# edwinb-ai/MolecularDynamics.jl

Hardware: AMD Instinct MI355X
Metric: particle-steps/sec + achieved HBM GB/s, 1M LJ particles rho=0.897, 1/2/4/8 GPUs (higher is better)
Workload: dtype f64; 1 GPU; BASELINE configs[2]: N=1048576 monodisperse LJ 3D rho=0.897 r_cut=2.5 dt=0.001 NVT Bussi tau=0.1 kT=1.4737, per GPU; particles_per_gpu=1048576, parallelism=1 GPU, step_loop=fused (k_step_tile: one launch per step + k_finalize), global_particles=1048576, tiled_force_kernel=True, max_tile_halo=2081, energies_every_step=False, thermo_frequency=2589

## Files before the change

### include/mdhip.h

```cpp
#ifndef MDHIP_H
#define MDHIP_H

#include <stdint.h>

#ifdef __cplusplus
extern "C" {
#endif

typedef struct md_ctx md_ctx;

enum { MD_POT_LJ = 0, MD_POT_PSEUDOHS = 1, MD_POT_POLYDISPERSE = 2, MD_POT_LJ_MODIFIED = 3, MD_POT_CUSTOM = 100 };

enum { MD_NVE = 0, MD_NVT = 1 };

int md_create(int dim, int64_t n_particles, const double *box, double list_cutoff, int device_id, md_ctx **out);
int md_destroy(md_ctx *ctx);

const char *md_last_error(md_ctx *ctx);

int md_set_potential(md_ctx *ctx, int kind, const double *params, int nparams);

int md_set_potential_source(md_ctx *ctx, const char *hip_src, const char *entry_name, const double *params,
                            int nparams);

int md_set_skin(md_ctx *ctx, double skin);

int md_set_inner_skin(md_ctx *ctx, double inner_skin);

int md_upload(md_ctx *ctx, const double *x, const double *v, const double *f, const int32_t *images,
              const double *diameters);
int md_download(md_ctx *ctx, double *x, double *v, double *f, int32_t *images);

int md_compute_forces(md_ctx *ctx, double *energy, double *virial);

int md_neighbor_pairs(md_ctx *ctx, int32_t *pairs, int64_t cap, int64_t *count);

int md_run(md_ctx *ctx, int64_t nsteps, double dt, int ensemble, double tau, double nf, const double *ktemp,
           const double *r1, const double *r2, double *uwk);

int md_fire_minimize(md_ctx *ctx, int64_t max_steps, double tol, double dt_initial, double dt_max, double alpha0,
                     double f_inc, double f_dec, int nmin, int64_t *steps, int *converged, double *energy,
                     double *f_rms);

int md_run_brownian(md_ctx *ctx, int64_t nsteps, double dt, double ktemp, uint64_t seed, int64_t first_step,
                    int64_t virial_every, double *out );

int md_snapshot_begin(md_ctx *ctx);
int md_snapshot_end(md_ctx *ctx, double *x, int32_t *images);

int md_rdf_setup(md_ctx *ctx, double r_max, int nbins);
int md_rdf_sample(md_ctx *ctx);
int md_rdf_read(md_ctx *ctx, int64_t *counts, int64_t *nsamples);
int md_rdf_reset(md_ctx *ctx);

int md_dyn_setup(md_ctx *ctx, int nslots, int nrows, const double *q, int nq, double r_max, int nbins);
int md_dyn_origin(md_ctx *ctx, int slot);
int md_dyn_sample(md_ctx *ctx, const int32_t *slots, const int32_t *rows, int count);
int md_dyn_read(md_ctx *ctx, int64_t *nsamples, double *sums, int64_t *hist);
int md_dyn_reset(md_ctx *ctx);

int md_sq_setup(md_ctx *ctx, const int32_t *n, int nvec, int nslots, int nrows);
int md_sq_sample(md_ctx *ctx, int add_static, const int32_t *slots, const int32_t *rows, int count, int origin_slot);
int md_sq_rho(md_ctx *ctx, double *rho);
int md_sq_read(md_ctx *ctx, int64_t *nstatic, double *s2, int64_t *nsamples, double *corr);
int md_sq_reset(md_ctx *ctx);

int md_kinetic(md_ctx *ctx, double *kinetic);

int md_scale_velocities(md_ctx *ctx, double s);

typedef struct {
    int64_t steps;
    int64_t rebuilds;
    int64_t violations;
    int64_t n_ghost;
    int64_t max_neighbors;
    double avg_neighbors;
    int64_t force_launches;
    double force_ms;
    int64_t max_halo;
    int64_t tiled;
    int64_t prunes;
    int64_t kickdrift_launches;
    double kickdrift_ms;
    int64_t fused;
    int64_t walked_outer;
    int64_t walked_inner;
    int64_t prune_launches_timed;
    double prune_ms;
    int64_t rebuilds_timed;
    double rebuild_ms;
    int64_t fused_build;
} md_stats;
int md_profile(md_ctx *ctx, int enable);
int md_get_stats(md_ctx *ctx, md_stats *out);

int md_create_domain(int dim, int64_t n_global, int64_t n_cap, const double *box, double list_cutoff,
                     int device_id, int rank, int nranks, md_ctx **out);
int md_dom_set_uniform(md_ctx *ctx, int uniform, double sigma);
int md_dom_upload(md_ctx *ctx, int64_t n_own, const int32_t *ids, const double *x, const double *v, const double *f,
                  const int32_t *images, const double *diameters);
int md_dom_download(md_ctx *ctx, int64_t cap, int64_t *n_own, int32_t *ids, double *x, double *v, double *f,
                    int32_t *images);
int md_dom_migrate_pack(md_ctx *ctx, int64_t *nsend );
int md_dom_migrate_unpack(md_ctx *ctx, const int64_t *nrecv );
int md_dom_halo_pack(md_ctx *ctx, int64_t *nsend );
int md_dom_halo_unpack(md_ctx *ctx, const int64_t *nrecv );
int md_dom_build(md_ctx *ctx);
int md_dom_set_step_buffers(md_ctx *ctx, void *send_left, void *send_right, void *recv_left, void *recv_right,
                            int64_t capacity_doubles);
int md_dom_get_sendbuf(md_ctx *ctx, int side, int64_t ndoubles, void *dst, int dst_is_device);
int md_dom_put_recvbuf(md_ctx *ctx, int side, int64_t ndoubles, const void *src, int src_is_device);
int md_dom_step_begin(md_ctx *ctx, double dt, int *violated);
int md_dom_step_end(md_ctx *ctx, double dt, int want_uw, double *uwk);
int md_dom_forces(md_ctx *ctx, double dt, int kick, int want_uw, double *uwk);
int md_dom_set_scale(md_ctx *ctx, double scale);
int md_dom_counts(md_ctx *ctx, int64_t *out );

int md_set_stream(md_ctx *ctx, void *hip_stream);
int md_dom_async_begin(md_ctx *ctx, int64_t nsteps, double dt, int ensemble, double tau, double nf, const double *ktemp,
                       const double *r1, const double *r2, int64_t prune_interval, void *flag_dev ,
                       void *kuw_dev );
int md_dom_step_a(md_ctx *ctx, double dt, int step);
int md_dom_step_b(md_ctx *ctx, double dt, int step, int want_uw);
int md_dom_step_c(md_ctx *ctx, int step, int want_uw);
int md_dom_async_end(md_ctx *ctx, int apply_pending_scale, int32_t *first_viol, double *uwk, double *info );

int md_dom_comm_unique_id(const char *rccl_path, void *id128);
int md_dom_comm_init(md_ctx *ctx, const char *rccl_path, const void *id128);
int md_dom_rebuild(md_ctx *ctx);
int md_dom_run_window(md_ctx *ctx, int64_t nsteps, double dt, int ensemble, double tau, double nf, const double *ktemp,
                      const double *r1, const double *r2, int report_last, int apply_pending_scale,
                      int64_t prune_interval, int32_t *first_viol, double *uwk, double *info );
int md_dom_enable_pruning(md_ctx *ctx, int on);
int md_dom_max_disp0(md_ctx *ctx, double *d0);
int md_dom_invalidate_inner(md_ctx *ctx);

const char *md_version(void);

#ifdef __cplusplus
}
#endif
#endif
```

### moleculardynamics/jl_amd/_lib.py

```python
import ctypes as C
import os

_HERE = os.path.dirname(os.path.abspath(__file__))
SO_PATH = os.path.join(_HERE, "csrc", "libmdhip.so")

MD_POT_LJ, MD_POT_PSEUDOHS, MD_POT_POLYDISPERSE, MD_POT_LJ_MODIFIED, MD_POT_CUSTOM = 0, 1, 2, 3, 100
MD_NVE, MD_NVT = 0, 1

EXPORTS = [
    "md_create", "md_destroy", "md_last_error", "md_set_potential", "md_set_potential_source", "md_set_skin",
    "md_set_inner_skin",
    "md_upload", "md_download", "md_snapshot_begin", "md_snapshot_end", "md_compute_forces", "md_neighbor_pairs", "md_run", "md_kinetic",
    "md_scale_velocities", "md_profile", "md_get_stats", "md_version", "md_fire_minimize", "md_run_brownian",
    "md_create_domain", "md_dom_set_uniform", "md_dom_upload", "md_dom_download", "md_dom_migrate_pack",
    "md_dom_migrate_unpack", "md_dom_halo_pack", "md_dom_halo_unpack", "md_dom_build", "md_dom_get_sendbuf",
    "md_dom_put_recvbuf", "md_dom_set_step_buffers", "md_dom_step_begin", "md_dom_step_end", "md_dom_forces", "md_dom_set_scale",
    "md_dom_counts", "md_set_stream", "md_dom_async_begin", "md_dom_step_a", "md_dom_step_b", "md_dom_step_c",
    "md_dom_async_end", "md_dom_comm_unique_id", "md_dom_comm_init", "md_dom_run_window", "md_dom_rebuild",
    "md_dom_enable_pruning", "md_dom_max_disp0", "md_dom_invalidate_inner",
    "md_rdf_setup", "md_rdf_sample", "md_rdf_read", "md_rdf_reset",
    "md_dyn_setup", "md_dyn_origin", "md_dyn_sample", "md_dyn_read", "md_dyn_reset",
    "md_sq_setup", "md_sq_sample", "md_sq_rho", "md_sq_read", "md_sq_reset",
]


class MdStats(C.Structure):
    _fields_ = [("steps", C.c_int64), ("rebuilds", C.c_int64), ("violations", C.c_int64), ("n_ghost", C.c_int64),
                ("max_neighbors", C.c_int64), ("avg_neighbors", C.c_double), ("force_launches", C.c_int64),
                ("force_ms", C.c_double), ("max_halo", C.c_int64), ("tiled", C.c_int64), ("prunes", C.c_int64),
                ("kickdrift_launches", C.c_int64), ("kickdrift_ms", C.c_double), ("fused", C.c_int64),
                ("walked_outer", C.c_int64), ("walked_inner", C.c_int64), ("prune_launches_timed", C.c_int64),
                ("prune_ms", C.c_double), ("rebuilds_timed", C.c_int64), ("rebuild_ms", C.c_double),
                ("fused_build", C.c_int64)]


class MdhipError(RuntimeError):
    pass


_lib = None


def load():
    global _lib
    if _lib is not None:
        return _lib
    if not os.path.exists(SO_PATH):
        raise MdhipError(
            f"{SO_PATH} not found: build it with `python -c 'import __graft_entry__ as g; g.build()'` or "
            "`make -C moleculardynamics/jl_amd/csrc`. There is no CPU fallback.")
    L = C.CDLL(SO_PATH)
    vp, dp, ip = C.c_void_p, C.POINTER(C.c_double), C.POINTER(C.c_int32)
    L.md_create.argtypes = [C.c_int, C.c_int64, dp, C.c_double, C.c_int, C.POINTER(vp)]
    L.md_create.restype = C.c_int
    L.md_destroy.argtypes = [vp]
    L.md_destroy.restype = C.c_int
    L.md_last_error.argtypes = [vp]
    L.md_last_error.restype = C.c_char_p
    L.md_set_potential.argtypes = [vp, C.c_int, dp, C.c_int]
    L.md_set_potential.restype = C.c_int
    L.md_set_potential_source.argtypes = [vp, C.c_char_p, C.c_char_p, dp, C.c_int]
    L.md_set_potential_source.restype = C.c_int
    L.md_set_skin.argtypes = [vp, C.c_double]
    L.md_set_skin.restype = C.c_int
    L.md_set_inner_skin.argtypes = [vp, C.c_double]
    L.md_set_inner_skin.restype = C.c_int
    L.md_upload.argtypes = [vp, dp, dp, dp, ip, dp]
    L.md_upload.restype = C.c_int
    L.md_download.argtypes = [vp, dp, dp, dp, ip]
    L.md_download.restype = C.c_int
    L.md_snapshot_begin.argtypes = [vp]
    L.md_snapshot_begin.restype = C.c_int
    L.md_snapshot_end.argtypes = [vp, dp, ip]
    L.md_snapshot_end.restype = C.c_int
    L.md_compute_forces.argtypes = [vp, dp, dp]
    L.md_compute_forces.restype = C.c_int
    L.md_neighbor_pairs.argtypes = [vp, ip, C.c_int64, C.POINTER(C.c_int64)]
    L.md_neighbor_pairs.restype = C.c_int
    L.md_run.argtypes = [vp, C.c_int64, C.c_double, C.c_int, C.c_double, C.c_double, dp, dp, dp, dp]
    L.md_run.restype = C.c_int
    L.md_kinetic.argtypes = [vp, dp]
    L.md_kinetic.restype = C.c_int
    L.md_scale_velocities.argtypes = [vp, C.c_double]
    L.md_scale_velocities.restype = C.c_int
    L.md_profile.argtypes = [vp, C.c_int]
    L.md_profile.restype = C.c_int
    L.md_get_stats.argtypes = [vp, C.POINTER(MdStats)]
    L.md_get_stats.restype = C.c_int
    L.md_version.argtypes = []
    L.md_version.restype = C.c_char_p
    i64p = C.POINTER(C.c_int64)
    L.md_create_domain.argtypes = [C.c_int, C.c_int64, C.c_int64, dp, C.c_double, C.c_int, C.c_int, C.c_int,
                                   C.POINTER(vp)]
    L.md_run_brownian.restype = C.c_int
    L.md_run_brownian.argtypes = [vp, C.c_int64, C.c_double, C.c_double, C.c_uint64, C.c_int64, C.c_int64, dp]
    L.md_fire_minimize.restype = C.c_int
    L.md_fire_minimize.argtypes = [vp, C.c_int64, C.c_double, C.c_double, C.c_double, C.c_double, C.c_double, C.c_double,
                                   C.c_int, i64p, C.POINTER(C.c_int), dp, dp]
    L.md_dom_set_uniform.argtypes = [vp, C.c_int, C.c_double]
    L.md_dom_upload.argtypes = [vp, C.c_int64, ip, dp, dp, dp, ip, dp]
    L.md_dom_download.argtypes = [vp, C.c_int64, i64p, ip, dp, dp, dp, ip]
    L.md_dom_migrate_pack.argtypes = [vp, i64p]
    L.md_dom_migrate_unpack.argtypes = [vp, i64p]
    L.md_dom_halo_pack.argtypes = [vp, i64p]
    L.md_dom_halo_unpack.argtypes = [vp, i64p]
    L.md_dom_build.argtypes = [vp]
    L.md_dom_rebuild.argtypes = [vp]
    L.md_dom_get_sendbuf.argtypes = [vp, C.c_int, C.c_int64, C.c_void_p, C.c_int]
    L.md_dom_put_recvbuf.argtypes = [vp, C.c_int, C.c_int64, C.c_void_p, C.c_int]
    L.md_dom_set_step_buffers.argtypes = [vp, C.c_void_p, C.c_void_p, C.c_void_p, C.c_void_p, C.c_int64]
    L.md_dom_step_begin.argtypes = [vp, C.c_double, C.POINTER(C.c_int)]
    L.md_dom_step_end.argtypes = [vp, C.c_double, C.c_int, dp]
    L.md_dom_forces.argtypes = [vp, C.c_double, C.c_int, C.c_int, dp]
    L.md_dom_set_scale.argtypes = [vp, C.c_double]
    L.md_dom_counts.argtypes = [vp, i64p]
    L.md_set_stream.argtypes = [vp, C.c_void_p]
    L.md_dom_async_begin.argtypes = [vp, C.c_int64, C.c_double, C.c_int, C.c_double, C.c_double, dp, dp, dp, C.c_int64,
                                     C.c_void_p, C.c_void_p]
    L.md_dom_step_a.argtypes = [vp, C.c_double, C.c_int]
    L.md_dom_step_b.argtypes = [vp, C.c_double, C.c_int, C.c_int]
    L.md_dom_step_c.argtypes = [vp, C.c_int, C.c_int]
    L.md_dom_async_end.argtypes = [vp, C.c_int, C.POINTER(C.c_int32), dp, dp]
    L.md_dom_comm_unique_id.argtypes = [C.c_char_p, C.c_void_p]
    L.md_dom_comm_init.argtypes = [vp, C.c_char_p, C.c_void_p]
    L.md_dom_run_window.argtypes = [vp, C.c_int64, C.c_double, C.c_int, C.c_double, C.c_double, dp, dp, dp, C.c_int, C.c_int,
                                    C.c_int64, C.POINTER(C.c_int32), dp, dp]
    L.md_dom_enable_pruning.argtypes = [vp, C.c_int]
    L.md_dom_max_disp0.argtypes = [vp, dp]
    L.md_dom_invalidate_inner.argtypes = [vp]
    L.md_rdf_setup.argtypes = [vp, C.c_double, C.c_int]
    L.md_rdf_setup.restype = C.c_int
    L.md_rdf_sample.argtypes = [vp]
    L.md_rdf_sample.restype = C.c_int
    L.md_rdf_read.argtypes = [vp, i64p, i64p]
    L.md_rdf_read.restype = C.c_int
    L.md_rdf_reset.argtypes = [vp]
    L.md_rdf_reset.restype = C.c_int
    L.md_dyn_setup.argtypes = [vp, C.c_int, C.c_int, dp, C.c_int, C.c_double, C.c_int]
    L.md_dyn_setup.restype = C.c_int
    L.md_dyn_origin.argtypes = [vp, C.c_int]
    L.md_dyn_origin.restype = C.c_int
    L.md_dyn_sample.argtypes = [vp, ip, ip, C.c_int]
    L.md_dyn_sample.restype = C.c_int
    L.md_dyn_read.argtypes = [vp, i64p, dp, i64p]
    L.md_dyn_read.restype = C.c_int
    L.md_dyn_reset.argtypes = [vp]
    L.md_dyn_reset.restype = C.c_int
    L.md_sq_setup.argtypes = [vp, ip, C.c_int, C.c_int, C.c_int]
    L.md_sq_setup.restype = C.c_int
    L.md_sq_sample.argtypes = [vp, C.c_int, ip, ip, C.c_int, C.c_int]
    L.md_sq_sample.restype = C.c_int
    L.md_sq_rho.argtypes = [vp, dp]
    L.md_sq_rho.restype = C.c_int
    L.md_sq_read.argtypes = [vp, i64p, dp, i64p, dp]
    L.md_sq_read.restype = C.c_int
    L.md_sq_reset.argtypes = [vp]
    L.md_sq_reset.restype = C.c_int
    for name in EXPORTS:
        if name.startswith("md_dom_") or name in ("md_create_domain", "md_set_stream"):
            getattr(L, name).restype = C.c_int
    _lib = L
    return L
```

### moleculardynamics/jl_amd/csrc/md_kernels.hpp

```cpp
#ifndef MD_RTC
#pragma once
#include <hip/hip_runtime.h>
#include <stdint.h>
#else
typedef __hip_internal::uint64_t uint64_t;
typedef __hip_internal::uint32_t uint32_t;
typedef __hip_internal::int32_t int32_t;
typedef __hip_internal::uint16_t uint16_t;
#endif

#define MD_BLOCK 256
#define MD_WAVE 64
#define MD_SENTINEL_POS 1.0e100
#define MD_VAL_SRC_BITS 26
#define MD_VAL_SRC_MASK ((1u << MD_VAL_SRC_BITS) - 1u)
#define MD_NO_VIOLATION 0x7fffffff

enum { POT_LJ = 0, POT_PSEUDOHS = 1, POT_POLYDISPERSE = 2, POT_LJ_MOD = 3, POT_CUSTOM = 100 };

struct DevState {
    double4 *pos;
    double *v[3];
    double *f[3];
    int32_t *img[3];
    int32_t *id;
    double *x0[3];
    double *x1[3];
    double boxL[3];
    int tric;
    double cellA[9];
};

struct BoxGrid {
    double L[3], invL[3];
    double lo[3];
    int selfimg[3];
    double inv_cell[3];
    int nc[3];
    int ncx[3];
    int bd[3];
    int nb[3];
    int n_int_cells;
    int id_bits, cell_bits;
    int tric;
    double A[9], Ainv[9];
};

struct PotParams {
    double p[8];
    double c2;
    uint32_t c2_k;
    uint32_t pad_;
    double sig2u;
    double sig_u;
    double c48, c24, c4;
    double ljA, ljB;
};

struct Scalars {
    double U, W, K, scale, T;
    unsigned long long max_disp2_bits;
    int first_viol;
    int overflow;
    unsigned long long pair_count;
    int hmax;
    int halo_overflow;
    int dbg_rmax, dbg_smax;
    unsigned long long d1max2_bits;
    int comm_error;
};

__device__ __forceinline__ double md_rcp(double a)
{
    double r = __builtin_amdgcn_rcp(a);
    double e = __builtin_fma(-a, r, 1.0);
    r = __builtin_fma(r, e, r);
    e = __builtin_fma(-a, r, 1.0);
    r = __builtin_fma(r, e, r);
    return r;
}

__device__ __forceinline__ double md_rcp1(double a)
{
    double r = __builtin_amdgcn_rcp(a);
    double e = __builtin_fma(-a, r, 1.0);
    return __builtin_fma(r, e, r);
}

__device__ __forceinline__ double mask_d2(double d2, bool hit)
{
    int hi = __double2hiint(d2);
    int lo = __double2loint(d2);
    hi = hit ? hi : 0x7fe00000;
    return __hiloint2double(hi, lo);
}

template <int D>
__device__ __forceinline__ double d2_ref(double dx, double dy, double dz)
{
#pragma clang fp contract(off)
    double a = dx * dx;
    double b = dy * dy;
    double r = a + b;
    if constexpr (D == 3) {
        double c = dz * dz;
        r = r + c;
    }
    return r;
}

template <int D>
__device__ __forceinline__ void frac_of(double x, double y, double z, const double *Ainv, double *fr)
{
#pragma clang fp contract(off)
#pragma unroll
    for (int r = 0; r < 3; ++r) {
        if (r < D) {
            double a = Ainv[r * 3 + 0] * x + Ainv[r * 3 + 1] * y;
            if constexpr (D == 3) a = a + Ainv[r * 3 + 2] * z;
            fr[r] = a;
        } else {
            fr[r] = 0.0;
        }
    }
}
template <int D>
__device__ __forceinline__ bool wrap_general(double &x, double &y, double &z, const double *A, const double *Ainv, int32_t *dn)
{
#pragma clang fp contract(off)
    double fr[3];
    frac_of<D>(x, y, z, Ainv, fr);
    bool out = false;
#pragma unroll
    for (int r = 0; r < D; ++r) out = out || fr[r] < 0.0 || fr[r] >= 1.0;
    dn[0] = dn[1] = dn[2] = 0;
    if (!out) return false;
    double fm[3] = {0.0, 0.0, 0.0};
#pragma unroll
    for (int r = 0; r < D; ++r) {
        double nn = floor(fr[r]);
        fm[r] = fr[r] - nn;
        dn[r] = (int32_t)nn;
    }
    double o[3] = {x, y, z};
#pragma unroll
    for (int r = 0; r < D; ++r) {
        double a = A[r * 3 + 0] * fm[0] + A[r * 3 + 1] * fm[1];
        if constexpr (D == 3) a = a + A[r * 3 + 2] * fm[2];
        o[r] = a;
    }
    x = o[0];
    y = o[1];
    if constexpr (D == 3) z = o[2];
    return true;
}
__device__ __forceinline__ void shift_xyz(double &x, double &y, double &z, uint32_t code, const double *L, int tric, const double *A)
{
#pragma clang fp contract(off)
    (void)L;
    (void)tric;
    const uint32_t sx = code & 3u, sy = (code >> 2) & 3u, sz = (code >> 4) & 3u;
    const double s0 = sx == 1u ? 1.0 : (sx == 2u ? -1.0 : 0.0);
    const double s1 = sy == 1u ? 1.0 : (sy == 2u ? -1.0 : 0.0);
    const double s2 = sz == 1u ? 1.0 : (sz == 2u ? -1.0 : 0.0);
    x = x + ((s0 * A[0] + s1 * A[1]) + s2 * A[2]);
    y = y + ((s0 * A[3] + s1 * A[4]) + s2 * A[5]);
    z = z + ((s0 * A[6] + s1 * A[7]) + s2 * A[8]);
}

__device__ __forceinline__ size_t row_off(int r, int lane) { return ((size_t)(r >> 2) * 64 + lane) * 4 + (r & 3); }

__device__ __forceinline__ double md_ipow(double x, int n)
{
    double r = 1.0;
    while (n) {
        if (n & 1) r *= x;
        x *= x;
        n >>= 1;
    }
    return r;
// ... 264 lines not shown
{
#pragma unroll
    for (int c = 0; c < 3; ++c) {
        e[c] = 0;
        b[c] = 0;
    }
    int cc3[3];
    cell_coords<D>(p, g, cc3);
#pragma unroll
    for (int c = 0; c < D; ++c) {
        double xc = pos_get(p, c);
        if (is_xh && !g.selfimg[c]) {
            e[c] = (xc < g.lo[c]) ? 0 : g.nc[c] + 1;
            continue;
        }
        int cc = cc3[c];
        e[c] = cc + 1;
        if (g.selfimg[c]) b[c] = (cc == 0) ? 1 : ((cc == g.nc[c] - 1) ? 2 : 0);
    }
}

template <int D>
__global__ void __launch_bounds__(MD_BLOCK)
    k_wrap_count(int n_src, int n_own_src, DevState s, BoxGrid g, const int32_t *__restrict__ alive,
                 int32_t *__restrict__ nimg)
{
    int i = blockIdx.x * blockDim.x + threadIdx.x;
    if (i >= n_src) return;
    if (i == 0) nimg[n_src] = 0;
    if (alive && !alive[i]) {
        nimg[i] = 0;
        return;
    }
    bool is_xh = i >= n_own_src;
    double4 p = s.pos[i];
    if (!is_xh) {
        bool moved = false;
        if (g.tric) {
            int32_t dn[3];
            moved = wrap_general<D>(p.x, p.y, p.z, g.A, g.Ainv, dn);
            if (moved) {
#pragma unroll
                for (int c = 0; c < D; ++c) s.img[c][i] += dn[c];
            }
        } else {
#pragma unroll
            for (int c = 0; c < D; ++c) {
                double xc = pos_get(p, c);
                if (xc < 0.0 || xc >= g.L[c]) {
                    double frac = g.invL[c] * xc;
                    double nn = floor(frac);
                    double fm = frac - nn;
                    s.img[c][i] += (int32_t)nn;
                    xc = g.L[c] * fm;
                    pos_set(p, c, xc);
                    moved = true;
                }
            }
        }
        if (moved) s.pos[i] = p;
    }
    int e[3], b[3];
    source_cells<D>(p, is_xh, g, e, b);
    int cnt = 1;
#pragma unroll
    for (int c = 0; c < D; ++c)
        if (b[c]) cnt *= 2;
    nimg[i] = cnt;
}

template <int D>
__global__ void __launch_bounds__(MD_BLOCK)
    k_emit(int n_src, int n_own_src, DevState s, BoxGrid g, const int32_t *__restrict__ alive,
           const int32_t *__restrict__ img_off, uint64_t *__restrict__ keys, uint32_t *__restrict__ vals,
           int32_t *__restrict__ cell_start, int32_t *__restrict__ cell_end, int ncell1)
{
    int i = blockIdx.x * blockDim.x + threadIdx.x;
    for (int j = i; j < ncell1; j += gridDim.x * blockDim.x) {
        cell_start[j] = 0;
        cell_end[j] = 0;
    }
    if (i >= n_src) return;
    if (alive && !alive[i]) return;
    bool is_xh = i >= n_own_src;
    double4 p = s.pos[i];
    int eb[3], b[3];
    source_cells<D>(p, is_xh, g, eb, b);
    uint64_t idv = (uint64_t)(uint32_t)s.id[i];
    uint64_t gbit = 1ull << (g.id_bits + g.cell_bits);
    int slot = img_off[i];
    for (int m = 0; m < (1 << D); ++m) {
        bool ok = true;
        uint32_t code = 0;
        int e[3] = {eb[0], eb[1], eb[2]};
#pragma unroll
        for (int c = 0; c < D; ++c) {
            if ((m >> c) & 1) {
                if (b[c] == 0) ok = false;
                e[c] = (b[c] == 1) ? g.nc[c] + 1 : 0;
                code |= (uint32_t)b[c] << (2 * c);
            }
        }
        if (!ok) continue;
        bool ghost = is_xh || m != 0;
        keys[slot] = (ghost ? gbit : 0ull) | ((uint64_t)ext_linear(e, g) << g.id_bits) | idv;
        vals[slot] = (uint32_t)i | (code << MD_VAL_SRC_BITS);
        ++slot;
    }
}

__device__ __forceinline__ double4 shifted(double4 p, uint32_t code, const BoxGrid &g)
{
    if (code) shift_xyz(p.x, p.y, p.z, code, g.L, g.tric, g.A);
    return p;
}

__device__ __forceinline__ void reset_flags(Scalars *sc)
{
    sc->first_viol = MD_NO_VIOLATION;
    sc->max_disp2_bits = 0ull;
    sc->overflow = 0;
    sc->hmax = 0;
    sc->halo_overflow = 0;
    sc->dbg_rmax = 0;
    sc->dbg_smax = 0;
    sc->d1max2_bits = 0ull;
}

template <int D>
__global__ void __launch_bounds__(MD_BLOCK)
    k_gather(int n, int next, DevState so, DevState sn, BoxGrid g, const uint64_t *__restrict__ keys,
             const uint32_t *__restrict__ vals, int32_t *__restrict__ newslot, int32_t *__restrict__ gsrc,
             uint32_t *__restrict__ gcode, int32_t *__restrict__ cell_start, int32_t *__restrict__ cell_end,
             Scalars *sc)
{
    int k = blockIdx.x * blockDim.x + threadIdx.x;
    if (k >= next) return;
    if (k == 0) reset_flags(sc);
    uint64_t key = keys[k];
    uint32_t val = vals[k];
    int src = (int)(val & MD_VAL_SRC_MASK);
    uint32_t code = val >> MD_VAL_SRC_BITS;
    double4 p = shifted(so.pos[src], code, g);
    sn.pos[k] = p;
    sn.id[k] = so.id[src];
    if (k < n) {
#pragma unroll
        for (int c = 0; c < D; ++c) {
            sn.v[c][k] = so.v[c][src];
            sn.f[c][k] = so.f[c][src];
            sn.img[c][k] = so.img[c][src];
            sn.x0[c][k] = pos_get(p, c);
        }
    } else {
        gsrc[k - n] = src;
        gcode[k - n] = code;
    }
    if (code == 0u) newslot[src] = k;
    uint64_t cmask = (1ull << (g.cell_bits + 1)) - 1ull;
    int ce = (int)((key >> g.id_bits) & cmask);
    int cprev = (k > 0) ? (int)((keys[k - 1] >> g.id_bits) & cmask) : -1;
    int cellmask = (1 << g.cell_bits) - 1;
    if (ce != cprev) {
        cell_start[ce & cellmask] = k;
        if (k > 0) cell_end[cprev & cellmask] = k;
    }
    if (k == next - 1) cell_end[ce & cellmask] = next;
}

__global__ void __launch_bounds__(MD_BLOCK)
    k_ghost_owner(int nghost, const int32_t *__restrict__ gsrc, const int32_t *__restrict__ newslot,
                  int32_t *__restrict__ gowner)
{
    int gi = blockIdx.x * blockDim.x + threadIdx.x;
    if (gi >= nghost) return;
    gowner[gi] = newslot[gsrc[gi]];
}

__global__ void __launch_bounds__(MD_BLOCK)
    k_halo_virtualize(int n, uint32_t *__restrict__ halo, int hcap, const int32_t *__restrict__ halo_count,
                      const int32_t *__restrict__ gowner, const uint32_t *__restrict__ gcode)
{
    uint32_t *hl = halo + (size_t)blockIdx.x * hcap;
    int H = halo_count[blockIdx.x];
    for (int h = threadIdx.x; h < H; h += blockDim.x) {
        uint32_t e = hl[h];
        if (e >= (uint32_t)n) hl[h] = (uint32_t)gowner[e - n] | (gcode[e - n] << 26);
    }
}

template <int D>
__global__ void __launch_bounds__(MD_BLOCK)
    k_ghost_update(int n, int nghost, DevState s, BoxGrid g, const int32_t *__restrict__ gowner,
                   const uint32_t *__restrict__ gcode, const Scalars *__restrict__ sc, int step)
{
    int gi = blockIdx.x * blockDim.x + threadIdx.x;
    if (gi >= nghost) return;
    if (sc->first_viol <= step) return;
    s.pos[n + gi] = shifted(s.pos[gowner[gi]], gcode[gi], g);
}

template <int D>
__global__ void __launch_bounds__(MD_BLOCK)
    k_build_list(int n, DevState s, BoxGrid g, double rl2, const int32_t *__restrict__ cell_start,
                 const int32_t *__restrict__ cell_end, uint32_t *__restrict__ nlist, int maxn,
                 int32_t *__restrict__ nneigh, int32_t *__restrict__ nmax_tile, uint32_t sentinel, Scalars *sc)
{
    int k = blockIdx.x * blockDim.x + threadIdx.x;
    bool active = k < n;
    int lane = threadIdx.x & 63;
    int tile = k >> 6;
    uint32_t *row = nlist + ((size_t)tile * maxn) * 64 + lane;
    const double4 *__restrict__ P = s.pos;
    int cnt = 0;
    if (active) {
        double4 pi = P[k];
        int ec[3];
        cell_coords<D>(pi, g, ec);
#pragma unroll
        for (int c = 0; c < D; ++c) ec[c] += 1;
        int z0 = (D == 3) ? -1 : 0, z1 = (D == 3) ? 1 : 0;
        for (int dz = z0; dz <= z1; ++dz)
            for (int dy = -1; dy <= 1; ++dy)
                for (int dx = -1; dx <= 1; ++dx) {
                    int e[3] = {ec[0] + dx, ec[1] + dy, (D == 3) ? ec[2] + dz : 0};
                    int cell = ext_linear(e, g);
                    int js = cell_start[cell], je = cell_end[cell];
                    for (int j = js; j < je; ++j) {
                        double4 pj = P[j];
                        double ddx = pj.x - pi.x;
                        double ddy = pj.y - pi.y;
                        double d2 = ddx * ddx;
                        d2 = __builtin_fma(ddy, ddy, d2);
                        if constexpr (D == 3) {
                            double ddz = pj.z - pi.z;
                            d2 = __builtin_fma(ddz, ddz, d2);
                        }
                        if (d2 <= rl2 && j != k) {
                            if (cnt < maxn) row[(size_t)cnt * 64] = (uint32_t)j;
                            ++cnt;
                        }
                    }
                }
        nneigh[k] = cnt;
        if (cnt > maxn) {
            atomicOr(&sc->overflow, 1);
            cnt = maxn;
        }
    }
    int m = wave_max_i(cnt);
    m = (m + 3) & ~3;
    if (m > maxn) m = maxn;
    for (int t = cnt; t < m; ++t) row[(size_t)t * 64] = sentinel;
    if (lane == 0) nmax_tile[tile] = m;
}

template <int D, int POT, bool UNIFORM, bool WANT_UW, bool KICK>
__global__ void __launch_bounds__(MD_BLOCK)
    k_force(int n, DevState s, PotParams pp, const uint32_t *__restrict__ nlist, int maxn,
            const int32_t *__restrict__ nmax_tile, double dt, double *__restrict__ partials, int nblk_total,
            const Scalars *__restrict__ sc, int step)
{
    __shared__ double red[16];
    if (sc->first_viol <= step) return;
    int bid = xcd_remap(blockIdx.x, gridDim.x);
    int k = bid * MD_BLOCK + threadIdx.x;
    bool active = k < n;
    int kk = active ? k : n - 1;
    int lane = threadIdx.x & 63;
    int tile = kk >> 6;
    const uint32_t *row = nlist + ((size_t)tile * maxn) * 64 + lane;
    int m = nmax_tile[tile];
    const double4 *__restrict__ P = s.pos;
    double4 pi = P[kk];
    double fx = 0.0, fy = 0.0, fz = 0.0, us = 0.0, ws = 0.0;
    for (int r = 0; r < m; r += 4) {
        uint32_t j[4];
#pragma unroll
        for (int q = 0; q < 4; ++q) j[q] = row[(size_t)(r + q) * 64];
        double4 pj[4];
#pragma unroll
        for (int q = 0; q < 4; ++q) pj[q] = P[j[q]];
#pragma unroll
        for (int q = 0; q < 4; ++q) {
            double dx = pj[q].x - pi.x;
            double dy = pj[q].y - pi.y;
            double dz = 0.0;
            if constexpr (D == 3) dz = pj[q].z - pi.z;
            double d2 = d2_ref<D>(dx, dy, dz);
            bool hit = d2 < pp.c2;
            double d2m = mask_d2(d2, hit);
            double u = 0.0, fpr;
            pair_eval<POT, UNIFORM, WANT_UW>(d2m, pi.w, pj[q].w, pp, u, fpr);
            fx = __builtin_fma(-fpr, dx, fx);
            fy = __builtin_fma(-fpr, dy, fy);
            if constexpr (D == 3) fz = __builtin_fma(-fpr, dz, fz);
            if constexpr (WANT_UW) {
                us += u;
                ws = __builtin_fma(fpr, hit ? d2 : 0.0, ws);
            }
        }
    }
    double ke = 0.0;
    if (active) {
        s.f[0][k] = fx;
        s.f[1][k] = fy;
// ... 85 lines not shown
            if (run < hcap) halo[(size_t)tile * hcap + run] = key;
            ++run;
        }
    }
    if (tid == 0) {
        halo_count[tile] = H;
        atomicMax(&sc->hmax, H);
        if (H > hcap || (H + 1) * rs > 65535) atomicOr(&sc->halo_overflow, 1);
    }
    __syncthreads();
    uint16_t *row16 = nlist16 + ((size_t)wt * maxn) * 64;
    for (int r = 0; r < m; ++r) {
        uint32_t j = row[(size_t)r * 64];
        uint32_t loc;
        if (j == sentinel) {
            loc = (uint32_t)H;
        } else {
            uint32_t h = (j * 2654435761u) >> (32 - MD_HT_BITS);
            while (keys[h] != j) h = (h + 1) & (MD_HT - 1);
            loc = vals[h];
        }
        row16[row_off(r, lane)] = (uint16_t)(loc * (uint32_t)rs);
    }
}

#ifndef MD_RTC
#include "md_build_tile.hpp"
#endif

struct PruneRow {
    unsigned char *base;
    unsigned off;
};
__device__ __forceinline__ void prune_append(unsigned entry, PruneRow &pr, unsigned long long &acc, int &cin)
{
    unsigned lo = (unsigned)acc, hi = (unsigned)(acc >> 32);
    lo = __builtin_amdgcn_alignbit(hi, lo, 16);
    hi = __builtin_amdgcn_alignbit(entry, hi, 16);
    acc = ((unsigned long long)hi << 32) | lo;
    ++cin;
    if ((cin & 3) == 0) {
        *(unsigned long long *)(pr.base + pr.off) = acc;
        pr.off += 512u;
    }
}

template <int D, int POT, bool UNIFORM, bool WANT_UW, bool PRUNE, int NQ>
__device__ __forceinline__ void tile_pair_block(const unsigned char *smem, const unsigned (&o)[NQ], const double4 &pi,
                                                const PotParams &pp, PruneRow &rin64, double rin2,
                                                unsigned long long &acc, int &cin, double &fx, double &fy, double &fz,
                                                double &us, double &ws, const uint16_t *remap8)
{
    double xj[NQ], yj[NQ], zj[NQ], wj[NQ];
#pragma unroll
    for (int q = 0; q < NQ; ++q) {
        typedef const volatile __attribute__((address_space(3))) double lds_cvd;
        if constexpr (!UNIFORM && D == 3) {
            typedef double md_d2 __attribute__((ext_vector_type(2)));
            typedef const __attribute__((address_space(3))) md_d2 lds_d2;
            lds_d2 *r2 = (lds_d2 *)(smem + o[q]);
            md_d2 a = r2[0], b = r2[1];
            xj[q] = a.x;
            yj[q] = a.y;
            zj[q] = b.x;
            wj[q] = b.y;
        } else {
            lds_cvd *rec = (lds_cvd *)(smem + o[q]);
            xj[q] = rec[0];
            yj[q] = rec[1];
            if constexpr (D == 3) zj[q] = rec[2];
            if constexpr (!UNIFORM) wj[q] = rec[3];
        }
    }
    if constexpr (POT == POT_LJ && UNIFORM && !WANT_UW && D == 3) {
        double dxq[NQ], dyq[NQ], dzq[NQ], dm[NQ];
        unsigned tmin = 0xffffffffu;
        double d2k[PRUNE ? NQ : 1];
#pragma unroll
        for (int q = 0; q < NQ; ++q) {
            dxq[q] = xj[q] - pi.x;
            dyq[q] = yj[q] - pi.y;
            dzq[q] = zj[q] - pi.z;
            double d2 = dxq[q] * dxq[q];
            d2 = __builtin_fma(dyq[q], dyq[q], d2);
            d2 = __builtin_fma(dzq[q], dzq[q], d2);
            if constexpr (PRUNE) d2k[q] = d2;
            int hi = __double2hiint(d2);
            unsigned t = (unsigned)hi - pp.c2_k;
            tmin = min(tmin, t);
            hi = ((int)t < 0) ? hi : 0x5fe00000;
            dm[q] = __hiloint2double(hi, __double2loint(d2));
        }
        if constexpr (PRUNE) {
#pragma unroll
            for (int q = 0; q < NQ; ++q) asm volatile("" : "+v"(d2k[q]));
#pragma unroll
            for (int q = 0; q < NQ; ++q)
                if (d2k[q] <= rin2)
                    prune_append(remap8 ? (unsigned)remap8[o[q] >> 3] : o[q], rin64, acc, cin);
        }
        if (__any(tmin <= 2u)) {
#pragma unroll
            for (int q = 0; q < NQ; ++q) {
                double d2 = dxq[q] * dxq[q];
                d2 = __builtin_fma(dyq[q], dyq[q], d2);
                d2 = __builtin_fma(dzq[q], dzq[q], d2);
                unsigned t = (unsigned)__double2hiint(d2) - pp.c2_k;
                if (t <= 2u) {
                    bool hit = d2_ref<3>(dxq[q], dyq[q], dzq[q]) < pp.c2;
                    dm[q] = __hiloint2double(hit ? __double2hiint(d2) : 0x5fe00000, __double2loint(d2));
                }
            }
        }
#pragma unroll
        for (int q = 0; q < NQ; q += 2) {
            double ip = md_rcp1(dm[q] * dm[q + 1]);
            double z[2] = {dm[q + 1] * ip, dm[q] * ip};
#pragma unroll
            for (int h = 0; h < 2; ++h) {
                double z2 = z[h] * z[h];
                double t = __builtin_fma(pp.ljA, z2 * z[h], -pp.ljB);
                double fpr = (z2 * z2) * t;
                fx = __builtin_fma(-fpr, dxq[q + h], fx);
                fy = __builtin_fma(-fpr, dyq[q + h], fy);
                fz = __builtin_fma(-fpr, dzq[q + h], fz);
            }
        }
    } else
#pragma unroll
    for (int q = 0; q < NQ; ++q) {
        double dx = xj[q] - pi.x;
        double dy = yj[q] - pi.y;
        double dz = 0.0;
        if constexpr (D == 3) dz = zj[q] - pi.z;
        double d2 = d2_ref<D>(dx, dy, dz);
        if constexpr (PRUNE) {
            if (d2 <= rin2)
                prune_append(remap8 ? (unsigned)remap8[o[q] >> 3] : o[q], rin64, acc, cin);
        }
        bool hit = d2 < pp.c2;
        double d2m = mask_d2(d2, hit);
        double u = 0.0, fpr;
        pair_eval<POT, UNIFORM, WANT_UW>(d2m, pi.w, UNIFORM ? 0.0 : wj[q], pp, u, fpr);
        fx = __builtin_fma(-fpr, dx, fx);
        fy = __builtin_fma(-fpr, dy, fy);
        if constexpr (D == 3) fz = __builtin_fma(-fpr, dz, fz);
        if constexpr (WANT_UW) {
            us += u;
            ws = __builtin_fma(fpr, hit ? d2 : 0.0, ws);
        }
    }
}

template <int D, int POT, bool UNIFORM, bool WANT_UW, bool PRUNE>
__device__ __forceinline__ void tile_pair_loop(const unsigned char *smem, const ushort4 *row4,
                                               ushort4 (&jn)[MD_UNROLL / 4], int m_lane, int H,
                                               const double4 &pi, const PotParams &pp, PruneRow &rin64,
                                               double rin2, unsigned long long &acc, int &cin, double &fx, double &fy,
                                               double &fz, double &us, double &ws, const uint16_t *remap8 = nullptr)
{
    constexpr int G = MD_UNROLL / 4;
    static_assert(G == 2, "the tail handling below assumes two groups per iteration");
    (void)H;
    const int m = __builtin_amdgcn_readfirstlane(m_lane);
    int r = 0;
    for (; r + MD_UNROLL <= m; r += MD_UNROLL) {
        unsigned o[MD_UNROLL];
#pragma unroll
        for (int g = 0; g < G; ++g) {
            o[4 * g + 0] = jn[g].x;
            o[4 * g + 1] = jn[g].y;
            o[4 * g + 2] = jn[g].z;
            o[4 * g + 3] = jn[g].w;
        }
#pragma unroll
        for (int g = 0; g < G; ++g) {
            int rg = r + MD_UNROLL + 4 * g;
            jn[g] = row4[(size_t)(((rg < m) ? rg : 0) >> 2) * 64];
        }
        tile_pair_block<D, POT, UNIFORM, WANT_UW, PRUNE, MD_UNROLL>(smem, o, pi, pp, rin64, rin2, acc, cin, fx, fy, fz, us,
                                                                     ws, remap8);
    }
    if (r < m) {
        unsigned o[4] = {jn[0].x, jn[0].y, jn[0].z, jn[0].w};
        tile_pair_block<D, POT, UNIFORM, WANT_UW, PRUNE, 4>(smem, o, pi, pp, rin64, rin2, acc, cin, fx, fy, fz, us, ws,
                                                            remap8);
    }
}

template <int D, bool UNIFORM>
__device__ __forceinline__ void tile_prune_tail(DevState &s, Scalars *sc, int H , int k, bool active, int lane, int wt,
                                                const double4 &pi, PruneRow rin64, int32_t *nmax_in,
                                                unsigned long long acc, int cin)
{
    constexpr int RS = UNIFORM ? 24 : 32;
    {
        const unsigned long long sent = (unsigned long long)(H * RS);
        const unsigned long long sent4 = sent | (sent << 16) | (sent << 32) | (sent << 48);
        int mw = wave_max_i((cin + 3) & ~3);
        int g = cin >> 2;
        if (cin & 3) {
            int p = cin & 3;
            *(unsigned long long *)(rin64.base + rin64.off) = (acc >> (16 * (4 - p))) | (sent4 << (16 * p));
            rin64.off += 512u;
            ++g;
        }
        for (; g < (mw >> 2); ++g, rin64.off += 512u) *(unsigned long long *)(rin64.base + rin64.off) = sent4;
        if (lane == 0) nmax_in[wt] = mw;
        double dd = 0.0;
        if (active) {
#pragma unroll
            for (int c = 0; c < D; ++c) {
                double xc = pos_get(pi, c);
                s.x1[c][k] = xc;
                double d = xc - s.x0[c][k];
                dd = __builtin_fma(d, d, dd);
            }
        }
        double wm = wave_max_d(dd);
        if (lane == 0 && wm > 0.0) atomicMax(&sc->d1max2_bits, (unsigned long long)__double_as_longlong(wm));
    }
}

template <int D, bool UNIFORM>
__device__ __forceinline__ int tile_inner_halo(unsigned char *smem, int H, const uint32_t *hl, int bid, const double4 &pi,
                                               bool active, double rin2, uint32_t *__restrict__ halo_in, int hcap_in,
                                               int32_t *__restrict__ halo_in_count, Scalars *sc, int step,
                                               const uint16_t **remap_out)
{
    constexpr int RS = UNIFORM ? 24 : 32;
    __shared__ double sh_bb[MD_TILE / 64][6];
    __shared__ int sh_scan2[16];
    __shared__ int sh_hin;
    const int lane = threadIdx.x & 63;
    uint16_t *rm = (uint16_t *)(smem + ((((size_t)(H + 1) * RS) + 15) & ~(size_t)15));
    const double big = 1.0e300;
    const double xn[3] = {pi.x, pi.y, pi.z};
    double lo3[3], hi3[3];
#pragma unroll
    for (int c = 0; c < 3; ++c) {
        double v = (c < D) ? xn[c] : 0.0;
        lo3[c] = -wave_max_d((active && c < D) ? -v : -big);
        hi3[c] = wave_max_d((active && c < D) ? v : -big);
    }
    if (lane == 0) {
#pragma unroll
        for (int c = 0; c < 3; ++c) {
            sh_bb[threadIdx.x >> 6][c] = lo3[c];
            sh_bb[threadIdx.x >> 6][3 + c] = hi3[c];
        }
    }
    __syncthreads();
#pragma unroll
    for (int c = 0; c < 3; ++c) {
        lo3[c] = big;
        hi3[c] = -big;
        for (int w = 0; w < MD_TILE / 64; ++w) {
            lo3[c] = fmin(lo3[c], sh_bb[w][c]);
            hi3[c] = fmax(hi3[c], sh_bb[w][3 + c]);
        }
    }
    int carry = 0;
    for (int h0 = 0; h0 < H; h0 += 8 * MD_TILE) {
        const int hb = h0 + 8 * (int)threadIdx.x;
        unsigned near = 0u;
#pragma unroll
        for (int i = 0; i < 8; ++i) {
            int h = hb + i;
            if (h < H) {
                const double *rec = (const double *)(smem + (size_t)h * RS);
                double dd = 0.0;
#pragma unroll
                for (int c = 0; c < D; ++c) {
                    double xc = rec[c];
                    double dl = fmax(fmax(lo3[c] - xc, xc - hi3[c]), 0.0);
                    dd = __builtin_fma(dl, dl, dd);
                }
                if (dd <= rin2) near |= 1u << i;
            }
        }
        int tot;
        int base = carry + block_excl_scan(__popc(near), sh_scan2, &tot);
#pragma unroll
        for (int i = 0; i < 8; ++i) {
            int h = hb + i;
            if (h < H) {
                bool nr = (near >> i) & 1u;
                rm[((unsigned)h * RS) >> 3] = nr ? (uint16_t)((unsigned)base * RS) : (uint16_t)0xffffu;
                if (nr) {
                    if (base < hcap_in) halo_in[(size_t)bid * hcap_in + base] = hl[h];
                    ++base;
                }
            }
        }
        carry += tot;
        __syncthreads();
    }
    if (threadIdx.x == 0) {
        sh_hin = carry;
        halo_in_count[bid] = carry;
        if (carry > hcap_in || (size_t)(carry + 1) * RS > 65535) {
            atomicOr(&sc->halo_overflow, 16);
            atomicMin(&sc->first_viol, step + 1);
        }
    }
    __syncthreads();
    *remap_out = rm;
    return sh_hin;
}

template <int D, int POT, bool UNIFORM, bool WANT_UW, bool KICK, bool PRUNE>
__global__ void __launch_bounds__(MD_TILE)
    k_force_tile(int n, DevState s, PotParams pp, const uint16_t *__restrict__ nlist16, int maxn,
                 const int32_t *__restrict__ nmax_tile, const uint32_t *__restrict__ halo, int hcap,
                 const int32_t *__restrict__ halo_count, double dt, double *__restrict__ partials, int nblk_total,
                 Scalars *__restrict__ sc, int step, uint16_t *__restrict__ rows_in, int32_t *__restrict__ nmax_in,
                 double rin2, long long *__restrict__ stamps = nullptr, uint32_t *__restrict__ halo_in = nullptr,
                 int hcap_in = 0, int32_t *__restrict__ halo_in_count = nullptr)
{
#define MD_SSTAMP(i)                                                                                   \
    do {                                                                                               \
        if (stamps && (threadIdx.x & 63) == 0)                                                         \
            stamps[((size_t)blockIdx.x * 4 + (threadIdx.x >> 6)) * 8 + (i)] = (long long)clock64();   \
    } while (0)
    constexpr int RS = UNIFORM ? 24 : 32;
    extern __shared__ __attribute__((aligned(16))) unsigned char smem[];
    __shared__ double red[16];
    if (sc->first_viol <= step) return;
    MD_SSTAMP(0);
    int bid = xcd_remap(blockIdx.x, gridDim.x);
    const double4 *__restrict__ P = s.pos;
    int H = halo_count[bid];
    const uint32_t *hl = halo + (size_t)bid * hcap;
    int k = bid * MD_TILE + threadIdx.x;
    bool active = k < n;
    int kk = active ? k : n - 1;
    int lane = threadIdx.x & 63;
    int wt = bid * (MD_TILE / 64) + (threadIdx.x >> 6);
    const ushort4 *row4 = (const ushort4 *)(nlist16 + ((size_t)wt * maxn) * 64) + lane;
    PruneRow rin64;
    rin64.base = PRUNE ? (unsigned char *)(rows_in + ((size_t)__builtin_amdgcn_readfirstlane(wt) * maxn) * 64) : nullptr;
    rin64.off = (unsigned)lane * 8u;
    unsigned long long acc = 0ull;
    int cin = 0;
    int m = nmax_tile[wt];
    double4 pi = P[kk];
    constexpr int G = MD_UNROLL / 4;
    ushort4 jn[G];
#pragma unroll
    for (int g = 0; g < G; ++g) jn[g] = row4[(size_t)((4 * g < m) ? g : 0) * 64];
    double v0[3] = {0.0, 0.0, 0.0};
    if constexpr (KICK) {
#pragma unroll
        for (int c = 0; c < D; ++c) v0[c] = s.v[c][kk];
    }
    MD_SSTAMP(1);
    for (int h0 = 0; h0 <= H; h0 += 8 * MD_TILE) {
        uint32_t idx[8];
#pragma unroll
        for (int i = 0; i < 8; ++i) {
            int h = h0 + i * MD_TILE + threadIdx.x;
            idx[i] = (h < H) ? hl[h] : 0xffffffffu;
        }
        double4 pr[8];
#pragma unroll
        for (int i = 0; i < 8; ++i)
            pr[i] = (idx[i] != 0xffffffffu) ? P[idx[i] & 0x3ffffffu]
                                            : make_double4(MD_SENTINEL_POS, MD_SENTINEL_POS, MD_SENTINEL_POS, 1.0);
#pragma unroll
        for (int i = 0; i < 8; ++i) {
            uint32_t code = (idx[i] != 0xffffffffu) ? (idx[i] >> 26) : 0u;
            if (code) shift_xyz(pr[i].x, pr[i].y, pr[i].z, code, s.boxL, s.tric, s.cellA);
        }
#pragma unroll
        for (int i = 0; i < 8; ++i) {
            int h = h0 + i * MD_TILE + threadIdx.x;
            if (h <= H) {
                double *rec = (double *)(smem + (size_t)h * RS);
                rec[0] = pr[i].x;
                rec[1] = pr[i].y;
                rec[2] = (D == 3) ? pr[i].z : 0.0;
                if constexpr (!UNIFORM) rec[3] = pr[i].w;
            }
        }
    }
    MD_SSTAMP(2);
    __syncthreads();
    MD_SSTAMP(3);
    const uint16_t *remap8 = nullptr;
    int Hsent = H;
    if constexpr (PRUNE) {
        if (halo_in)
            Hsent = tile_inner_halo<D, UNIFORM>(smem, H, hl, bid, pi, active, rin2, halo_in, hcap_in, halo_in_count, sc, step,
                                                &remap8);
    }
    double fx = 0.0, fy = 0.0, fz = 0.0, us = 0.0, ws = 0.0;
    tile_pair_loop<D, POT, UNIFORM, WANT_UW, PRUNE>(smem, row4, jn, m, H, pi, pp, rin64, rin2, acc, cin, fx, fy, fz, us, ws, remap8);
    MD_SSTAMP(4);
    if constexpr (PRUNE) tile_prune_tail<D, UNIFORM>(s, sc, Hsent, k, active, lane, wt, pi, rin64, nmax_in, acc, cin);
    double ke = 0.0;
    if (active) {
        s.f[0][k] = fx;
        s.f[1][k] = fy;
        if constexpr (D == 3) s.f[2][k] = fz;
        if constexpr (KICK) {
            double vx = v0[0] + (fx * dt) / 2.0;
            double vy = v0[1] + (fy * dt) / 2.0;
            s.v[0][k] = vx;
            s.v[1][k] = vy;
            ke = vx * vx + vy * vy;
            if constexpr (D == 3) {
                double vz = v0[2] + (fz * dt) / 2.0;
                s.v[2][k] = vz;
                ke += vz * vz;
            }
        }
    } else {
        us = 0.0;
        ws = 0.0;
    }
    if constexpr (KICK) {
        double t = block_sum(ke, red);
        if (threadIdx.x == 0) partials[bid] = t;
    }
    if constexpr (WANT_UW) {
        double tu = block_sum(us, red);
        double tw = block_sum(ws, red);
        if (threadIdx.x == 0) {
            partials[nblk_total + bid] = tu;
            partials[2 * nblk_total + bid] = tw;
        }
    }
    MD_SSTAMP(5);
#undef MD_SSTAMP
}

struct StepBufs {
    const double2 *recA;
    double2 *recB;
    size_t rstride;
    const double *fA[3];
    double *fB[3];
    double4 *posB;
};

template <int D, int POT, bool UNIFORM, bool WANT_UW, bool PRUNE>
__global__ void __launch_bounds__(MD_TILE)
    k_step_tile(int n, DevState s, StepBufs sb, PotParams pp, const uint16_t *__restrict__ nlist16, int maxn,
                const int32_t *__restrict__ nmax_tile, const uint32_t *__restrict__ halo, int hcap,
                const int32_t *__restrict__ halo_count, double dt, double skin_half, double inner_half, int use_d1,
                double *__restrict__ partials, int nblk_total, Scalars *__restrict__ sc, int step,
                uint16_t *__restrict__ rows_in, int32_t *__restrict__ nmax_in, double rin2,
                long long *__restrict__ stamps, uint32_t *__restrict__ halo_in, int hcap_in,
                int32_t *__restrict__ halo_in_count, const int32_t *__restrict__ tile_list = nullptr)
{
#define MD_SSTAMP(i)                                                                                   \
    do {                                                                                               \
        if (stamps && (threadIdx.x & 63) == 0)                                                         \
            stamps[((size_t)blockIdx.x * 4 + (threadIdx.x >> 6)) * 8 + (i)] = (long long)clock64();   \
    } while (0)
    constexpr int RS = UNIFORM ? 24 : 32;
    extern __shared__ __attribute__((aligned(16))) unsigned char smem[];
    __shared__ double red[16];
    if (sc->first_viol < step) return;
    MD_SSTAMP(0);
    int bid = xcd_remap(blockIdx.x, gridDim.x);
    if (tile_list) bid = tile_list[bid];
    int H = halo_count[bid];
    const uint32_t *hl = halo + (size_t)bid * hcap;
    int k = bid * MD_TILE + threadIdx.x;
    bool active = k < n;
    int kk = active ? k : n - 1;
    int lane = threadIdx.x & 63;
    int wt = bid * (MD_TILE / 64) + (threadIdx.x >> 6);
    const ushort4 *row4 = (const ushort4 *)(nlist16 + ((size_t)wt * maxn) * 64) + lane;
    PruneRow rin64;
    rin64.base = PRUNE ? (unsigned char *)(rows_in + ((size_t)__builtin_amdgcn_readfirstlane(wt) * maxn) * 64) : nullptr;
    rin64.off = (unsigned)lane * 8u;
    unsigned long long acc = 0ull;
    int cin = 0;
    int m = nmax_tile[wt];
    const double alpha = sc->scale;
    const double adt = alpha * dt;
    const double2 *RA0 = sb.recA, *RA1 = RA0 + sb.rstride, *RA2 = RA1 + sb.rstride, *RA3 = RA2 + sb.rstride;
    double2 a0 = RA0[kk], a1 = RA1[kk], a2 = RA2[kk];
    double sig_own = pp.sig_u;
    if constexpr (!UNIFORM) sig_own = RA3[kk].x;
    double fprev[3] = {0.0, 0.0, 0.0}, xr[3] = {0.0, 0.0, 0.0};
#pragma unroll
    for (int c = 0; c < D; ++c) {
        fprev[c] = sb.fA[c][kk];
        xr[c] = PRUNE ? s.x0[c][kk] : s.x1[c][kk];
    }
    constexpr int G = MD_UNROLL / 4;
    ushort4 jn[G];
#pragma unroll
    for (int g = 0; g < G; ++g) jn[g] = row4[(size_t)((4 * g < m) ? g : 0) * 64];
    MD_SSTAMP(1);
#ifndef MD_STAGE_NB
#define MD_STAGE_NB ((!PRUNE && UNIFORM && !WANT_UW) ? 6 : 8)
#endif
    constexpr int NB = MD_STAGE_NB;
    for (int h0 = 0; h0 <= H; h0 += NB * MD_TILE) {
        uint32_t idx[NB];
#pragma unroll
        for (int i = 0; i < NB; ++i) {
            int h = h0 + i * MD_TILE + threadIdx.x;
            idx[i] = (h < H) ? hl[h] : 0xffffffffu;
        }
        double2 r0[NB], r1[NB], r2[NB], r3[NB];
#pragma unroll
        for (int i = 0; i < NB; ++i) {
            bool ok = idx[i] != 0xffffffffu;
            size_t j = ok ? (size_t)(idx[i] & 0x3ffffffu) : 0;
            r0[i] = RA0[j];
            r1[i] = RA1[j];
            r2[i] = RA2[j];
            if constexpr (!UNIFORM) r3[i] = RA3[j];
        }
#pragma unroll
        for (int i = 0; i < NB; ++i) {
            int h = h0 + i * MD_TILE + threadIdx.x;
            bool ok = idx[i] != 0xffffffffu;
            double x = __builtin_fma(adt, r1[i].y, r0[i].x);
            double y = __builtin_fma(adt, r2[i].x, r0[i].y);
            double z = (D == 3) ? __builtin_fma(adt, r2[i].y, r1[i].x) : 0.0;
            uint32_t code = ok ? (idx[i] >> 26) : 0u;
            if (code) shift_xyz(x, y, z, code, s.boxL, s.tric, s.cellA);
            if (!ok) {
                x = MD_SENTINEL_POS;
                y = MD_SENTINEL_POS;
                z = (D == 3) ? MD_SENTINEL_POS : 0.0;
            }
            if (h <= H) {
                double *rec = (double *)(smem + (size_t)h * RS);
                rec[0] = x;
                rec[1] = y;
                rec[2] = z;
                if constexpr (!UNIFORM) rec[3] = ok ? r3[i].x : 1.0;
            }
        }
    }
    const double pown[3] = {a0.x, a0.y, a1.x}, vown[3] = {a1.y, a2.x, a2.y};
    double vh[3] = {0.0, 0.0, 0.0}, xn[3] = {0.0, 0.0, 0.0};
    double disp2 = 0.0;
#pragma unroll
    for (int c = 0; c < D; ++c) {
        vh[c] = alpha * vown[c] + (fprev[c] * dt) / 2.0;
        xn[c] = __builtin_fma(adt, vown[c], pown[c]);
        double d = xn[c] - xr[c];
        disp2 = __builtin_fma(d, d, disp2);
    }
    const double4 pi = make_double4(xn[0], xn[1], xn[2], sig_own);
    if (active) sb.posB[k] = pi;
    {
        double d1 = use_d1 ? sqrt(__longlong_as_double((long long)sc->d1max2_bits)) : 0.0;
        double thr = fmin(inner_half, skin_half - d1);
        double thr2 = thr > 0.0 ? thr * thr : -1.0;
        if (__any(active && disp2 > thr2)) {
            if (lane == 0) atomicMin(&sc->first_viol, step);
        }
    }
    MD_SSTAMP(2);
    __syncthreads();
    MD_SSTAMP(3);
    double fx = 0.0, fy = 0.0, fz = 0.0, us = 0.0, ws = 0.0;
    tile_pair_loop<D, POT, UNIFORM, WANT_UW, PRUNE>(smem, row4, jn, m, H, pi, pp, rin64, rin2, acc, cin, fx, fy, fz, us, ws, nullptr);
    MD_SSTAMP(4);
    if constexpr (PRUNE) tile_prune_tail<D, UNIFORM>(s, sc, H, k, active, lane, wt, pi, rin64, nmax_in, acc, cin);
    double ke = 0.0;
    if (active) {
        const double fn[3] = {fx, fy, fz};
        const double h2 = (dt * dt) / 2.0;
        double vp[3] = {0.0, 0.0, 0.0}, pn[3] = {0.0, 0.0, 0.0};
#pragma unroll
        for (int c = 0; c < D; ++c) {
            sb.fB[c][k] = fn[c];
            vp[c] = vh[c] + (fn[c] * dt) / 2.0;
            pn[c] = __builtin_fma(h2, fn[c], xn[c]);
            ke += vp[c] * vp[c];
        }
        double2 *RB = sb.recB;
        RB[k] = make_double2(pn[0], pn[1]);
        RB[sb.rstride + k] = make_double2(pn[2], vp[0]);
        RB[2 * sb.rstride + k] = make_double2(vp[1], vp[2]);
        if constexpr (!UNIFORM) RB[3 * sb.rstride + k] = make_double2(sig_own, 0.0);
    } else {
        us = 0.0;
        ws = 0.0;
    }
    {
        double t = block_sum(ke, red);
        if (threadIdx.x == 0) partials[bid] = t;
    }
    if constexpr (WANT_UW) {
        double tu = block_sum(us, red);
        double tw = block_sum(ws, red);
        if (threadIdx.x == 0) {
            partials[nblk_total + bid] = tu;
            partials[2 * nblk_total + bid] = tw;
        }
    }
    MD_SSTAMP(5);
#undef MD_SSTAMP
}

template <int D, bool UNIFORM>
__global__ void __launch_bounds__(MD_BLOCK) k_fuse(int n, DevState s, double2 *__restrict__ rec, size_t rstride, double h2)
{
    int k = blockIdx.x * blockDim.x + threadIdx.x;
    if (k >= n) return;
    double4 p = s.pos[k];
    double pp3[3] = {p.x, p.y, (D == 3) ? p.z : 0.0}, v3[3] = {0.0, 0.0, 0.0};
#pragma unroll
    for (int c = 0; c < D; ++c) {
        pp3[c] = __builtin_fma(h2, s.f[c][k], pp3[c]);
        v3[c] = s.v[c][k];
    }
    rec[k] = make_double2(pp3[0], pp3[1]);
    rec[rstride + k] = make_double2(pp3[2], v3[0]);
    rec[2 * rstride + k] = make_double2(v3[1], v3[2]);
    if constexpr (!UNIFORM) rec[3 * rstride + k] = make_double2(p.w, 0.0);
}

template <int D, bool UNIFORM>
__global__ void __launch_bounds__(MD_BLOCK)
    k_unfuse(int n, DevState s, const double2 *__restrict__ rec, size_t rstride, const Scalars *sc, int apply_scale)
{
    int k = blockIdx.x * blockDim.x + threadIdx.x;
    if (k >= n) return;
    double2 b1 = rec[rstride + k], b2 = rec[2 * rstride + k];
    const double v3[3] = {b1.y, b2.x, b2.y};
    double scale = apply_scale ? sc->scale : 1.0;
#pragma unroll
    for (int c = 0; c < D; ++c) s.v[c][k] = v3[c] * scale;
}

struct BussiSrc {
    const double *sums;
    const double *kt, *r1, *r2;
    double nf, term1;
    int idx;
};

template <int D, bool SCALE>
__global__ void __launch_bounds__(MD_BLOCK)
    k_kickdrift(int n, DevState s, double dt, double skin_half, double inner_half, int use_d1, Scalars *sc, int step,
                BussiSrc bs)
{
    if (sc->first_viol < step) return;
    int k = blockIdx.x * blockDim.x + threadIdx.x;
    double d1 = use_d1 ? sqrt(__longlong_as_double((long long)sc->d1max2_bits)) : 0.0;
    double thr = fmin(inner_half, skin_half - d1);
    double thr2 = thr > 0.0 ? thr * thr : -1.0;
    double disp2 = 0.0;
    if (k < n) {
        double scale = 1.0;
        if constexpr (SCALE) {
            if (bs.sums) {
                double K = bs.sums[0] / 2.0;
                double tc = 2.0 * K / bs.nf;
                double rr1 = bs.r1[bs.idx], rr2 = bs.r2[bs.idx];
                double c2 = (1.0 - bs.term1) * bs.kt[bs.idx] / (tc * bs.nf);
                double term_2 = c2 * (rr2 + rr1 * rr1);
                double term_3 = 2.0 * rr1 * sqrt(bs.term1 * c2);
                scale = sqrt(bs.term1 + term_2 + term_3);
            } else {
                scale = sc->scale;
            }
        }
        double4 p = s.pos[k];
#pragma unroll
        for (int c = 0; c < D; ++c) {
            double vc = s.v[c][k];
            if constexpr (SCALE) vc = vc * scale;
            vc = vc + (s.f[c][k] * dt) / 2.0;
            s.v[c][k] = vc;
            double xc = pos_get(p, c) + vc * dt;
            pos_set(p, c, xc);
            double d = xc - s.x1[c][k];
            disp2 = __builtin_fma(d, d, disp2);
        }
        s.pos[k] = p;
    }
    if (__any(disp2 > thr2)) {
        if ((threadIdx.x & 63) == 0) atomicMin(&sc->first_viol, step);
    }
}

template <int D>
__global__ void __launch_bounds__(MD_BLOCK) k_max_disp0(int n, DevState s, Scalars *sc)
{
    int k = blockIdx.x * blockDim.x + threadIdx.x;
    double dd = 0.0;
    if (k < n) {
        double4 p = s.pos[k];
#pragma unroll
        for (int c = 0; c < D; ++c) {
            double d = pos_get(p, c) - s.x0[c][k];
            dd = __builtin_fma(d, d, dd);
        }
    }
    double wm = wave_max_d(dd);
    if ((threadIdx.x & 63) == 0) {
        unsigned long long bits = (unsigned long long)__double_as_longlong(wm);
        if (bits > sc->max_disp2_bits) atomicMax(&sc->max_disp2_bits, bits);
    }
}

template <int D>
__global__ void __launch_bounds__(MD_BLOCK) k_scale_v(int n, DevState s, const Scalars *sc, double host_scale, int use_dev)
{
    int k = blockIdx.x * blockDim.x + threadIdx.x;
    if (k >= n) return;
    if (use_dev == 2 && sc->first_viol != MD_NO_VIOLATION) return;
    double scale = use_dev ? sc->scale : host_scale;
#pragma unroll
    for (int c = 0; c < D; ++c) s.v[c][k] = s.v[c][k] * scale;
}

template <int D>
__global__ void __launch_bounds__(MD_BLOCK) k_ke_partials(int n, DevState s, double *__restrict__ partials)
{
    __shared__ double red[16];
    int k = blockIdx.x * blockDim.x + threadIdx.x;
    double ke = 0.0;
    if (k < n) {
#pragma unroll
        for (int c = 0; c < D; ++c) ke += s.v[c][k] * s.v[c][k];
    }
    double t = block_sum(ke, red);
    if (threadIdx.x == 0) partials[blockIdx.x] = t;
}

__global__ void __launch_bounds__(1024)
    k_finalize(int nblk, const double *__restrict__ partials, int want_uw, int nvt, double nf, double term1,
               const double *__restrict__ kt, const double *__restrict__ r1, const double *__restrict__ r2,
               Scalars *sc, int step)
{
    __shared__ double red[16];
    if (sc->first_viol <= step) return;
    double a = strided_sum<4>(partials, nblk), b = 0.0, c = 0.0;
    if (want_uw) {
// ... 327 lines not shown
```

### moleculardynamics/jl_amd/csrc/mdhip.hip

```cpp
#include <cstring>
#include <cstdlib>
#include <unistd.h>

#include "md_kernels.hpp"
#include "md_domain.hpp"
#include "md_rdf.hpp"
#include "md_dyn.hpp"
#include "md_sq.hpp"

#include <rocprim/rocprim.hpp>

#include <algorithm>
#include <climits>
#include <cmath>
#include <cstdio>
#include <cstring>
#include <stdexcept>
#include <string>
#include <vector>

#include "../../../include/mdhip.h"
#include "md_rtc.hpp"
#include "md_rccl.hpp"

static RcclApi g_rccl;
static const bool g_dom_group_flag = [] { const char *e = getenv("MDHIP_DOM_GROUP_FLAG"); return e && e[0] == '1'; }();

namespace {

struct HipError : std::runtime_error {
    using std::runtime_error::runtime_error;
};

#define HIPCHK(expr)                                                                                        \
    do {                                                                                                    \
        hipError_t e_ = (expr);                                                                             \
        if (e_ != hipSuccess) {                                                                             \
            char buf_[512];                                                                                 \
            snprintf(buf_, sizeof buf_, "%s failed: %s (%s:%d)", #expr, hipGetErrorString(e_), __FILE__,    \
                     __LINE__);                                                                             \
            throw HipError(buf_);                                                                           \
        }                                                                                                   \
    } while (0)

template <class T>
struct DBuf {
    T *p = nullptr;
    size_t n = 0;
    void alloc(size_t count)
    {
        release();
        if (count == 0) count = 1;
        HIPCHK(hipMalloc((void **)&p, count * sizeof(T)));
        n = count;
    }
    void ensure(size_t count)
    {
        if (count > n) alloc(count + count / 4 + 16);
    }
    void release()
    {
        if (p) (void)hipFree(p);
        p = nullptr;
        n = 0;
    }
    ~DBuf() { release(); }
};

struct StateBufs {
    DBuf<double4> pos;
    DBuf<double> v[3], f[3], x0[3];
    DBuf<int32_t> img[3], id;
};

inline int ceil_log2(uint64_t v)
{
    int b = 0;
    while ((1ull << b) < v) ++b;
    return b;
}

std::string g_create_error;

}

struct md_ctx {
    int dim = 3;
    int64_t n = 0;
    int64_t ncap = 0;
    int64_t n_global = 0;
    int64_t src_count = 0;
    struct Domain {
        bool on = false;
        int rank = 0, nranks = 1;
        double xlo = 0.0, xhi = 0.0;
        int64_t n_old = 0, n_arr = 0, n_xh = 0;
        int64_t nsend_mig[2] = {0, 0}, nsend_halo[2] = {0, 0}, nrecv_halo[2] = {0, 0};
        DBuf<int32_t> alive, counters, hs_src[2], send_slot[2], xh_slot;
        DBuf<double> sbuf[2], rbuf[2];
        double *ext_send[2] = {nullptr, nullptr}, *ext_recv[2] = {nullptr, nullptr};
        int64_t ext_cap = 0;
        int32_t *flag_dev = nullptr;
        double *kuw_dev = nullptr;
        bool a_nvt = false;
        double a_nf = 0.0, a_term1 = 0.0;
        int64_t w_nsteps = 0, w_b0 = 0, w_prune_interval = 0;
        bool w_scale_from_sums = false;
        std::vector<int> w_prune_steps;
        ncclComm_t comm = nullptr;
        bool prune_enabled = false;
        DBuf<int32_t> own_flag;
        DBuf<int64_t> cnt_dev;
        DBuf<int32_t> tile_flag, tiles_b, tiles_i;
        int n_tiles_b = 0, n_tiles_i = 0;
        hipStream_t stream_i = nullptr;
        hipEvent_t ev_go = nullptr, ev_int = nullptr;
        DBuf<double> own_kuw;
        bool xhalo_pos_stale = false;
        struct P2p {
            bool on = false;
            char *mail = nullptr;
            int64_t cap = 0;
            char *peer[MD_P2P_MAXR] = {};
            bool opened[MD_P2P_MAXR] = {};
            int64_t peer_cap[MD_P2P_MAXR] = {};
            unsigned long long seq = 0;
            unsigned *done = nullptr;
            long long timeout = 0;
            bool window = false;
        } p2p;
    } dom;
    double L[3] = {1, 1, 1};
    int tric = 0;
    double A[9] = {1, 0, 0, 0, 1, 0, 0, 0, 1}, Ainv[9] = {1, 0, 0, 0, 1, 0, 0, 0, 1};
    double perp[3] = {1, 1, 1};
    double volume = 1.0;
    double rc = 0.0;
    double skin_req = 0.6;
    double skin = 0.0;
    double rl = 0.0;
    int pot_kind = POT_LJ;
    PotParams pp{};
    RtcModule *rtc = nullptr;
    bool uniform_sigma = true;
    double sigma_u = 1.0;
    int device = 0;
    hipStream_t stream = nullptr;
    hipStream_t own_stream = nullptr;

    int64_t cap = 0;
    int64_t next = 0;
    int64_t nghost = 0;
    StateBufs sb[2];
    int cur = 0;
    BoxGrid grid{};
    int ncell_ext = 0;

    DBuf<int32_t> nimg, img_off, newslot, gsrc, gowner, cell_start, cell_end, nneigh, nmax_tile;
    DBuf<uint32_t> gcode, vals_in, vals_out, nlist, halo;
    DBuf<uint16_t> nlist16;
    DBuf<int32_t> halo_count;
    DBuf<long long> dbg_stamps;
    int hcap = 4096;
    int hstride = 0;
    size_t tile_lds = 0;
    bool use_tiles = false;
    int tile_rs = 24;
    bool allow_tiles = true;
    bool allow_fused_build = true;
    bool have_nlist32 = false;
    DBuf<uint64_t> keys_in, keys_out;
    DBuf<char> sort_tmp, scan_tmp;
    int maxn = 0;
    int64_t ntiles = 0;

    DBuf<double> partials;
    DBuf<double> fire_part;
    DBuf<FireState> fire_state;
    DBuf<double> brown_acc;
    int nblk = 0;
    DBuf<Scalars> scal;
    DBuf<double> d_kt, d_r1, d_r2;

    DBuf<double> io_x, io_v, io_f, io_d;
    DBuf<int32_t> io_i;
    DBuf<double> snap_x;
    DBuf<int32_t> snap_i;
    double *pin_x = nullptr;
    int32_t *pin_i = nullptr;
    size_t pin_n = 0;
    hipStream_t copy_stream = nullptr;
    hipEvent_t ev_snap_ready = nullptr, ev_snap_copied = nullptr;
    bool snap_pending = false;

    bool list_valid = false;
    int64_t steps_since_build = 0;
    int64_t target_interval = 8;
    double inner_skin_req = 0.16;
    double inner_skin = 0.0;
    bool virtual_ghosts = false;
    bool inner_valid = false;
    bool prune_on = false;
    DBuf<double> x1[3];
    DBuf<uint16_t> nlist16_in;
    DBuf<int32_t> nmax_tile_in;
    int64_t steps_since_prune = 0;
    DBuf<double2> rec[2];
    DBuf<uint32_t> halo_in;
    DBuf<int32_t> halo_in_count;
    int hcap_in = 0;
    size_t tile_lds_in = 0;
    bool allow_inner_halo = true;
    bool inner_halo_live = false;
    int fz_a = 0;
    bool allow_fused = true;
    double d1_rate = 0.0;
    bool rate_known = false;
    double safety = 0.97;
    int64_t st_prunes = 0;

    int64_t st_steps = 0, st_rebuilds = 0, st_viol = 0;
    bool prof = false;
    int prof_stride = 1;
    int64_t prof_seen[2] = {0, 0};
    bool prof_open = false;
    std::vector<std::pair<hipEvent_t, hipEvent_t>> prof_ev;
    size_t prof_used = 0;
    double prof_ms_acc = 0.0;
    int64_t prof_launch_acc = 0;
    std::vector<int> prof_tag;
    double prof_kd_ms_acc = 0.0;
    int64_t prof_kd_launch_acc = 0;
    int64_t prof_prune_acc = 0;
    double prof_prune_ms_acc = 0.0;
    double prof_rebuild_ms_acc = 0.0;
    int64_t prof_rebuild_acc = 0;
    bool prof_cur_prune = false;
    bool last_run_fused = false;
    struct StepPart {
        const int32_t *list = nullptr;
        int count = 0;
        hipStream_t stream = nullptr;
        bool last = true;
    } part;

    struct Rdf {
        bool on = false;
        double r_max = 0.0;
        int nbins = 0;
        RdfGrid grid{};
        int64_t nsamples = 0;
        DBuf<double> e2;
        DBuf<unsigned long long> hist;
        DBuf<double4> wrec, srec;
        DBuf<uint32_t> keys_in, keys_out, vals_in, vals_out;
        DBuf<int32_t> cell_start, cell_end, work;
        DBuf<char> sort_tmp;
    } rdf;

    struct Dyn {
        bool on = false;
        int nslots = 0, nrows = 0, nq = 0, nbins = 0;
        double r_max = 0.0;
        std::vector<double> q;
        std::vector<char> filled;
        std::vector<int64_t> nsamples;
        double *ox = nullptr;
        int32_t *oi = nullptr;
        DBuf<double> cx, part, sums, e2;
        DBuf<int32_t> ci;
        DBuf<unsigned long long> hist;
        void release_slots()
        {
            if (ox) (void)hipFree(ox);
            if (oi) (void)hipFree(oi);
            ox = nullptr;
            oi = nullptr;
        }
        ~Dyn() { release_slots(); }
    } dyn;

    struct Sq {
        bool on = false;
        int nvec = 0, nvec_pad = 0, nslots = 0, nrows = 0, nblk = 0;
        bool sampled = false;
        int64_t nstatic = 0;
        std::vector<char> filled;
        std::vector<int64_t> nsamples;
        DBuf<double> nd;
        DBuf<double> cx, fr, part, rho, s2, corr, org;
        DBuf<int32_t> ci;
    } sq;

    std::string err;
    bool state_invalid = false;

    DevState dev(int which)
    {
        DevState s{};
        StateBufs &b = sb[which];
        s.pos = b.pos.p;
        for (int c = 0; c < 3; ++c) {
            s.v[c] = b.v[c].p;
            s.f[c] = b.f[c].p;
            s.img[c] = b.img[c].p;
            s.x0[c] = b.x0[c].p;
            s.x1[c] = (inner_valid && x1[c].p) ? x1[c].p : b.x0[c].p;
        }
        s.id = b.id.p;
        for (int c = 0; c < 3; ++c) s.boxL[c] = c < dim ? L[c] : 0.0;
        s.tric = tric;
        for (int c = 0; c < 9; ++c) s.cellA[c] = A[c];
        return s;
    }
};

namespace {

inline int nblocks(int64_t n) { return (int)((n + MD_BLOCK - 1) / MD_BLOCK); }

__global__ void k_init_state(int n, int64_t cap, DevState s, int dim)
{
    int64_t k = (int64_t)blockIdx.x * blockDim.x + threadIdx.x;
    if (k > cap) return;
    bool sent = (k == cap);
    double sp = sent ? MD_SENTINEL_POS : 0.0;
    s.pos[k] = make_double4(sp, sp, dim == 3 ? sp : 0.0, 1.0);
    s.id[k] = sent ? -1 : (k < n ? (int32_t)k : 0);
    if (k < n)
        for (int c = 0; c < dim; ++c) {
            s.v[c][k] = 0.0;
            s.f[c][k] = 0.0;
            s.img[c][k] = 0;
            s.x0[c][k] = 0.0;
        }
}

__global__ void k_reset_flags(Scalars *sc) { reset_flags(sc); }

__global__ void k_reset_disp0(Scalars *sc) { sc->max_disp2_bits = 0ull; }
__global__ void k_clear_halo_overflow(Scalars *sc) { sc->halo_overflow = 0; }

__global__ void k_reset_d1(Scalars *sc, int step)
{
    if (step >= 0 && sc->first_viol <= step) return;
    sc->d1max2_bits = 0ull;
}

void alloc_state(md_ctx *c, int which, int64_t cap)
{
    StateBufs &b = c->sb[which];
    b.pos.alloc(cap + 1);
    for (int d = 0; d < c->dim; ++d) {
        b.v[d].alloc(c->ncap);
        b.f[d].alloc(c->ncap);
        b.img[d].alloc(c->ncap);
        b.x0[d].alloc(c->ncap);
    }
    b.id.alloc(cap + 1);
}

struct CellGeom {
    int tric = 0;
    double A[9] = {1, 0, 0, 0, 1, 0, 0, 0, 1}, Ainv[9] = {1, 0, 0, 0, 1, 0, 0, 0, 1};
    double perp[3] = {1, 1, 1};
    double volume = 1.0;
};
const char *cell_geometry(int dim, const double *box, CellGeom &g)
{
#pragma clang fp contract(off)
    bool diag = true;
    for (int r = 0; r < dim; ++r)
        for (int c = 0; c < dim; ++c) {
            double v = box[c * dim + r];
            if (!std::isfinite(v)) return "md_create: unit cell entries must be finite";
            if (r != c && v != 0.0) diag = false;
            g.A[r * 3 + c] = v;
        }
    if (diag) {
        g.volume = 1.0;
        for (int c = 0; c < dim; ++c) {
            double v = g.A[c * 3 + c];
            if (!(v > 0.0)) return "md_create: box lengths must be positive";
            g.Ainv[c * 3 + c] = 1.0 / v;
            g.perp[c] = v;
            g.volume *= v;
        }
        g.tric = 0;
        return nullptr;
    }
    const double *U = g.A;
    double det;
    if (dim == 2) {
        det = U[0] * U[4] - U[1] * U[3];
        if (!(std::fabs(det) > 0.0) || !std::isfinite(det)) return "md_create: the unit cell matrix is singular";
        g.Ainv[0] = U[4] / det;
        g.Ainv[1] = -U[1] / det;
        g.Ainv[3] = -U[3] / det;
        g.Ainv[4] = U[0] / det;
    } else {
        double c00 = U[4] * U[8] - U[5] * U[7], c01 = U[5] * U[6] - U[3] * U[8], c02 = U[3] * U[7] - U[4] * U[6];
        det = (U[0] * c00 + U[1] * c01) + U[2] * c02;
        if (!(std::fabs(det) > 0.0) || !std::isfinite(det)) return "md_create: the unit cell matrix is singular";
        g.Ainv[0] = c00 / det;
        g.Ainv[1] = (U[2] * U[7] - U[1] * U[8]) / det;
        g.Ainv[2] = (U[1] * U[5] - U[2] * U[4]) / det;
        g.Ainv[3] = c01 / det;
        g.Ainv[4] = (U[0] * U[8] - U[2] * U[6]) / det;
        g.Ainv[5] = (U[2] * U[3] - U[0] * U[5]) / det;
        g.Ainv[6] = c02 / det;
        g.Ainv[7] = (U[1] * U[6] - U[0] * U[7]) / det;
        g.Ainv[8] = (U[0] * U[4] - U[1] * U[3]) / det;
    }
    for (int r = 0; r < dim; ++r) {
        double n2 = 0.0;
        for (int c = 0; c < dim; ++c) n2 += g.Ainv[r * 3 + c] * g.Ainv[r * 3 + c];
        g.perp[r] = 1.0 / std::sqrt(n2);
    }
    g.volume = std::fabs(det);
    g.tric = 1;
    return nullptr;
}

void configure_grid(md_ctx *c)
{
    double W[3] = {c->perp[0], c->perp[1], c->perp[2]};
    if (c->dom.on) W[0] = c->dom.xhi - c->dom.xlo;
    double lmin = 1e300;
    for (int d = 0; d < c->dim; ++d) {
        double need = (c->dom.on && d == 0) ? 2.0 : 3.0;
        lmin = std::min(lmin, W[d] / need);
    }
    if (lmin < c->rc) {
        char b[256];
        snprintf(b, sizeof b,
                 "box too small for the linked-cell build: need every box length (general cell: face distance) >= 3*list_cutoff (slab width >= "
                 "2*list_cutoff); got limit %g for list_cutoff=%g",
                 lmin, c->rc);
        throw HipError(b);
    }
    double skin = std::max(0.0, c->skin_req);
    double smax = lmin - c->rc;
    if (skin > smax) skin = std::max(0.0, smax * 0.999);
    c->skin = skin;
    c->rl = c->rc + skin;
    BoxGrid &g = c->grid;
    int64_t ncell = 1;
    for (int d = 0; d < 3; ++d) {
        g.lo[d] = 0.0;
        g.selfimg[d] = 1;
        if (d < c->dim) {
            g.L[d] = c->L[d];
            g.invL[d] = 1.0 / c->L[d];
            int kmin = (c->dom.on && d == 0) ? 2 : 3;
            int k = (int)std::floor(W[d] / c->rl);
            while (k > kmin && W[d] / k < c->rl) --k;
            if (k < kmin) k = kmin;
            g.nc[d] = k;
            g.ncx[d] = k + 2;
            g.inv_cell[d] = (double)k / W[d];
        } else {
            g.L[d] = 1.0;
            g.invL[d] = 1.0;
            g.nc[d] = 1;
            g.ncx[d] = 1;
            g.inv_cell[d] = 0.0;
        }
    }
    if (c->dom.on) {
        g.lo[0] = c->dom.xlo;
        g.selfimg[0] = 0;
    }
    g.tric = c->tric;
    for (int d = 0; d < 9; ++d) {
        g.A[d] = c->A[d];
        g.Ainv[d] = c->Ainv[d];
    }
    int target[3] = {2, 2, 3};
    if (c->dim == 2) {
        target[0] = 4; target[1] = 3; target[2] = 1;
    }
    int64_t nint = 1, next_plain = 1;
    for (int d = 0; d < 3; ++d) {
        g.nb[d] = std::max(1, g.nc[d] / target[d]);
        g.bd[d] = (g.nc[d] + g.nb[d] - 1) / g.nb[d];
        nint *= (int64_t)g.nb[d] * g.bd[d];
        next_plain *= g.ncx[d];
    }
    ncell = nint + next_plain;
    g.n_int_cells = (int)nint;
    if (ncell > (1ll << 30)) throw HipError("cell grid too large");
    c->ncell_ext = (int)ncell;
    g.id_bits = std::max(1, ceil_log2((uint64_t)std::max<int64_t>(c->n_global, 2)));
    g.cell_bits = std::max(1, ceil_log2((uint64_t)ncell));
    c->cell_start.ensure(ncell + 1);
    c->cell_end.ensure(ncell + 1);
    c->list_valid = false;
}

double sqrt_ge_threshold(double r)
{
    if (!(r > 0.0) || !std::isfinite(r)) return 0.0;
    double t = r * r;
    for (int i = 0; i < 64 && t > 0.0 && std::sqrt(t) >= r; ++i) t = std::nextafter(t, 0.0);
    for (int i = 0; i < 64 && std::sqrt(t) < r; ++i) t = std::nextafter(t, INFINITY);
    return t;
}

void configure_potential(md_ctx *c)
{
    double c2_incl = c->rc * c->rc;
    double c2 = std::nextafter(c2_incl, INFINITY);
// ... 79 lines not shown
    c->scan_tmp.ensure(tmp_bytes);
    HIPCHK(rocprim::exclusive_scan(c->scan_tmp.p, tmp_bytes, c->nimg.p, c->img_off.p, (int32_t)0, (size_t)n_src + 1,
                                   rocprim::plus<int32_t>(), st));
    int32_t total = 0;
    HIPCHK(hipMemcpyAsync(&total, c->img_off.p + n_src, sizeof(int32_t), hipMemcpyDeviceToHost, st));
    HIPCHK(hipStreamSynchronize(st));
    int64_t next = total;
    int n = (int)n_new;
    int32_t nghost = (int32_t)(next - n_new);
    if (nghost < 0) throw HipError("internal: fewer sort entries than owned particles");
    ensure_capacity(c, next);
    so = c->dev(c->cur);
    DevState sn = c->dev(c->cur ^ 1);

    k_emit<D><<<nbs, MD_BLOCK, 0, st>>>(n_src, n_own_src, so, g, alive, c->img_off.p, c->keys_in.p, c->vals_in.p,
                                        c->cell_start.p, c->cell_end.p, c->ncell_ext + 1);
    unsigned begin_bit = (unsigned)g.id_bits, end_bit = (unsigned)(g.id_bits + g.cell_bits + 1);
    tmp_bytes = 0;
    HIPCHK(rocprim::radix_sort_pairs(nullptr, tmp_bytes, c->keys_in.p, c->keys_out.p, c->vals_in.p, c->vals_out.p,
                                     (size_t)next, begin_bit, end_bit, st));
    c->sort_tmp.ensure(tmp_bytes);
    HIPCHK(rocprim::radix_sort_pairs(c->sort_tmp.p, tmp_bytes, c->keys_in.p, c->keys_out.p, c->vals_in.p,
                                     c->vals_out.p, (size_t)next, begin_bit, end_bit, st));
    k_gather<D><<<nblocks(next), MD_BLOCK, 0, st>>>(n, (int)next, so, sn, g, c->keys_out.p, c->vals_out.p,
                                                     c->newslot.p, c->gsrc.p, c->gcode.p, c->cell_start.p,
                                                     c->cell_end.p, c->scal.p);
    if (nghost > 0)
        k_ghost_owner<<<nblocks(nghost), MD_BLOCK, 0, st>>>(nghost, c->gsrc.p, c->newslot.p, c->gowner.p);
    c->cur ^= 1;
    c->next = next;
    c->nghost = nghost;
    c->n = n_new;
    c->nblk = nblocks(n_new);
    c->src_count = n_new;
    int nb = c->nblk;

    double rl2 = c->rl * c->rl;
    c->use_tiles = false;
    c->have_nlist32 = false;
    bool tile_ok = false;
    const int rs = (c->uniform_sigma && c->pot_kind != POT_POLYDISPERSE && c->pot_kind != POT_LJ_MOD && c->pot_kind != POT_CUSTOM) ? 24 : 32;
    auto set_tiles = [&](const Scalars &h) {
        size_t bytes = ((size_t)(h.hmax + 1) * rs + 15) & ~(size_t)15;
        if (!(h.halo_overflow) && bytes <= 150 * 1024) {
            c->use_tiles = true;
            c->hstride = h.hmax;
            c->tile_lds = bytes;
            c->tile_rs = rs;
            if (const char *e = getenv("MDHIP_LDS_PAD")) c->tile_lds += (size_t)atoi(e);
            return true;
        }
        return false;
    };
    auto grow_rows = [&]() {
        c->maxn = ((c->maxn * 3 / 2) + 3) & ~3;
        c->nlist.alloc((size_t)c->ntiles * c->maxn * 64);
        c->nlist16.alloc((size_t)c->ntiles * c->maxn * 64);
    };
    if (c->allow_tiles && c->allow_fused_build) {
        float rl2f = (float)(rl2 * (1.0 + 1.0e-4));
        for (int attempt = 0; attempt < 8; ++attempt) {
            if (attempt > 0 || next == 0) k_reset_flags<<<1, 1, 0, st>>>(c->scal.p);
            k_build_tile<D><<<c->nblk, MD_BT_THREADS, 0, st>>>(n, sn, g, rl2f, c->cell_start.p, c->cell_end.p,
                                                               c->nlist16.p, c->maxn, c->nneigh.p, c->nmax_tile.p,
                                                               c->halo.p, c->hcap, c->halo_count.p, c->scal.p,
                                                               c->dbg_stamps.p, rs);
            if (c->dbg_stamps.p) {
                std::vector<long long> hs((size_t)c->nblk * 10);
                HIPCHK(hipMemcpyAsync(hs.data(), c->dbg_stamps.p, hs.size() * 8, hipMemcpyDeviceToHost, st));
                HIPCHK(hipStreamSynchronize(st));
                double acc[9] = {0};
                for (int b = 0; b < c->nblk; ++b)
                    for (int i = 1; i <= 8; ++i) acc[i] += (double)(hs[(size_t)b * 10 + i] - hs[(size_t)b * 10 + i - 1]);
                fprintf(stderr, "[mdhip] build_tile phase cycles/block: cand %.0f sort %.0f uniq %.0f stage %.0f sweep0 %.0f compact %.0f sweep1 %.0f tail %.0f\n",
                        acc[1] / c->nblk, acc[2] / c->nblk, acc[3] / c->nblk, acc[4] / c->nblk, acc[5] / c->nblk,
                        acc[6] / c->nblk, acc[7] / c->nblk, acc[8] / c->nblk);
            }
            Scalars h;
            HIPCHK(hipMemcpyAsync(&h, c->scal.p, sizeof(Scalars), hipMemcpyDeviceToHost, st));
            HIPCHK(hipStreamSynchronize(st));
            if (getenv("MDHIP_DEBUG"))
                fprintf(stderr, "[mdhip] fused build: Rmax=%d Smax=%d Hmax=%d halo_overflow=%d row_overflow=%d maxn=%d\n",
                        h.dbg_rmax, h.dbg_smax, h.hmax, h.halo_overflow, h.overflow, c->maxn);
            if (h.halo_overflow) break;
            if (h.overflow) {
                grow_rows();
                continue;
            }
            tile_ok = set_tiles(h);
            break;
        }
    }
    if (!tile_ok) {
        for (int attempt = 0; attempt < 8; ++attempt) {
            k_reset_flags<<<1, 1, 0, st>>>(c->scal.p);
            k_build_list<D><<<nb, MD_BLOCK, 0, st>>>(n, sn, g, rl2, c->cell_start.p, c->cell_end.p, c->nlist.p,
                                                     c->maxn, c->nneigh.p, c->nmax_tile.p, (uint32_t)c->cap,
                                                     c->scal.p);
            Scalars h;
            HIPCHK(hipMemcpyAsync(&h, c->scal.p, sizeof(Scalars), hipMemcpyDeviceToHost, st));
            HIPCHK(hipStreamSynchronize(st));
            if (!h.overflow) break;
            if (attempt == 7) throw HipError("neighbour rows keep overflowing");
            grow_rows();
        }
        c->have_nlist32 = true;
        if (c->allow_tiles) {
            static int attr_dev_mask2 = 0;
            size_t lds = (size_t)MD_HT * 4 + (size_t)MD_HT * 2 + (MD_TILE + 1) * 4;
            if (!(attr_dev_mask2 & (1 << (c->device & 31)))) {
                HIPCHK(hipFuncSetAttribute((const void *)k_tile_localize, hipFuncAttributeMaxDynamicSharedMemorySize, (int)lds));
                attr_dev_mask2 |= 1 << (c->device & 31);
            }
            k_tile_localize<<<c->nblk, MD_TILE, lds, st>>>(c->nlist.p, c->nlist16.p, c->maxn, c->nmax_tile.p,
                                                           (uint32_t)c->cap, c->halo.p, c->hcap, c->halo_count.p,
                                                           c->scal.p, rs);
            Scalars h;
            HIPCHK(hipMemcpyAsync(&h, c->scal.p, sizeof(Scalars), hipMemcpyDeviceToHost, st));
            HIPCHK(hipStreamSynchronize(st));
            set_tiles(h);
        }
    }
    c->virtual_ghosts = c->use_tiles && c->cap < (1ll << 26);
    if (c->virtual_ghosts && nghost > 0)
        k_halo_virtualize<<<c->nblk, MD_BLOCK, 0, st>>>(n, c->halo.p, c->hcap, c->halo_count.p, c->gowner.p, c->gcode.p);
    if (getenv("MDHIP_ROWSTATS")) {
        std::vector<int32_t> nn((size_t)n), nm((size_t)c->ntiles);
        HIPCHK(hipMemcpyAsync(nn.data(), c->nneigh.p, sizeof(int32_t) * n, hipMemcpyDeviceToHost, st));
        HIPCHK(hipMemcpyAsync(nm.data(), c->nmax_tile.p, sizeof(int32_t) * c->ntiles, hipMemcpyDeviceToHost, st));
        HIPCHK(hipStreamSynchronize(st));
        double mean = 0, padded = 0, sorted_p = 0, p8 = 0, s8 = 0;
        for (int i = 0; i < n; ++i) mean += nn[i];
        for (int w = 0; w < (n + 63) / 64; ++w) { padded += nm[w]; p8 += (nm[w] + 7) & ~7; }
        for (int t0 = 0; t0 + 256 <= n; t0 += 256) {
            std::vector<int> v(nn.begin() + t0, nn.begin() + t0 + 256);
            std::sort(v.begin(), v.end());
            for (int w = 0; w < 4; ++w) { int mx = (v[64 * w + 63] + 3) & ~3; sorted_p += mx; s8 += (mx + 7) & ~7; }
        }
        int nw = (n + 63) / 64;
        fprintf(stderr, "[mdhip] rows: mean %.2f  wave-max(4) %.2f  wave-max(8) %.2f  sorted-within-tile(4) %.2f  (8) %.2f\n",
                mean / n, padded / nw, p8 / nw, sorted_p / nw, s8 / nw);
    }
    c->list_valid = true;
    c->steps_since_build = 0;
    c->st_rebuilds++;
    c->inner_valid = false;
    c->prune_on = c->use_tiles && (!c->dom.on || c->dom.prune_enabled) && c->skin > 0.0 && c->inner_skin_req > 0.0 &&
                  c->inner_skin_req < 0.9 * c->skin && c->pot_kind != POT_CUSTOM;
    if (c->prune_on) {
        c->inner_skin = c->inner_skin_req;
        for (int d = 0; d < c->dim; ++d) c->x1[d].ensure(c->ncap);
        c->nlist16_in.ensure((size_t)c->ntiles * c->maxn * 64);
        c->nmax_tile_in.ensure(c->ntiles);
        const size_t target = (c->tile_rs == 24) ? (40 * 1024 - 256) : (53 * 1024);
        int cap_in = (int)std::min<size_t>((size_t)c->hstride, target / c->tile_rs - 1);
        if (c->dom.on || getenv("MDHIP_INNER_CAP_OUTER")) cap_in = c->hstride;
        c->hcap_in = std::max(cap_in, 1);
        c->tile_lds_in = (((size_t)(c->hcap_in + 1) * c->tile_rs) + 15) & ~(size_t)15;
        c->halo_in.ensure((size_t)c->nblk * c->hcap_in);
        c->halo_in_count.ensure(c->nblk);
    }
}

void rebuild(md_ctx *c)
{
    if (c->dim == 3)
        rebuild_t<3>(c);
    else
        rebuild_t<2>(c);
    HIPCHK(hipGetLastError());
}

void prof_begin(md_ctx *c, int tag = 0)
{
    if (!c->prof) return;
    c->prof_open = tag >= 2 || (c->prof_seen[tag]++ % c->prof_stride) == 0;
    if (!c->prof_open) return;
    if (c->prof_used >= c->prof_ev.size()) {
        if (c->prof_ev.size() >= 8192) return;
        hipEvent_t a, b;
        HIPCHK(hipEventCreate(&a));
        HIPCHK(hipEventCreate(&b));
        c->prof_ev.emplace_back(a, b);
        c->prof_tag.push_back(0);
    }
    c->prof_tag[c->prof_used] = tag;
    HIPCHK(hipEventRecord(c->prof_ev[c->prof_used].first, c->stream));
}
void prof_end(md_ctx *c)
{
    if (!c->prof || !c->prof_open) return;
    c->prof_open = false;
    if (c->prof_used >= c->prof_ev.size()) return;
    HIPCHK(hipEventRecord(c->prof_ev[c->prof_used].second, c->stream));
    c->prof_used++;
}
void prof_collect(md_ctx *c)
{
    if (c->prof_used == 0) return;
    HIPCHK(hipStreamSynchronize(c->stream));
    for (size_t i = 0; i < c->prof_used; ++i) {
        float ms = 0.f;
        HIPCHK(hipEventElapsedTime(&ms, c->prof_ev[i].first, c->prof_ev[i].second));
        if (c->prof_tag[i] == 1) {
            c->prof_kd_ms_acc += ms;
            c->prof_kd_launch_acc++;
        } else if (c->prof_tag[i] == 2) {
            c->prof_rebuild_ms_acc += ms;
            c->prof_rebuild_acc++;
        } else if (c->prof_tag[i] == 3) {
            c->prof_prune_ms_acc += ms;
            c->prof_prune_acc++;
        } else {
            c->prof_ms_acc += ms;
            c->prof_launch_acc++;
        }
    }
    c->prof_used = 0;
}

template <int D, int POT, bool UNIFORM>
void launch_force_tpu(md_ctx *c, bool want_uw, bool kick, double dt, int step, int rows)
{
    int n = (int)c->n;
    int nb = c->nblk;
    bool prune_step = rows == 0 && c->prune_on && !c->inner_valid && kick;
    bool use_inner = rows == 0 && c->inner_valid;
    const uint16_t *rows16 = use_inner ? c->nlist16_in.p : c->nlist16.p;
    const int32_t *rowmax = use_inner ? c->nmax_tile_in.p : c->nmax_tile.p;
    const bool ih = c->allow_inner_halo && c->prune_on && c->hcap_in > 0 && c->use_tiles;
    const uint32_t *halo_p = c->halo.p;
    int halo_cap = c->hcap;
    const int32_t *halo_cnt = c->halo_count.p;
    size_t lds_bytes = c->tile_lds;
    uint32_t *hin_p = nullptr;
    if (prune_step && ih) {
        hin_p = c->halo_in.p;
        lds_bytes = ((c->tile_lds + 15) & ~(size_t)15) + (c->tile_lds / 8 + 8) * 2;
        c->inner_halo_live = true;
    } else if (prune_step) {
        c->inner_halo_live = false;
    } else if (use_inner && c->inner_halo_live) {
        halo_p = c->halo_in.p;
        halo_cap = c->hcap_in;
        halo_cnt = c->halo_in_count.p;
        lds_bytes = c->tile_lds_in;
    }
    DevState s = c->dev(c->cur);
    double rin = c->rc + c->inner_skin;
    if (prune_step) {
        for (int d = 0; d < 3; ++d) s.x1[d] = c->x1[d].p;
        k_reset_d1<<<1, 1, 0, c->stream>>>(c->scal.p, step);
    }
#define LF(UW, KK)                                                                                                  \
    k_force<D, POT, UNIFORM, UW, KK><<<nb, MD_BLOCK, 0, c->stream>>>(n, s, c->pp, c->nlist.p, c->maxn,              \
                                                                     c->nmax_tile.p, dt, c->partials.p, nb,         \
                                                                     c->scal.p, step)
#define LT(UW, KK, PR)                                                                                              \
    do {                                                                                                            \
        static int attr_dev_mask = 0;                       \
        auto kfn = k_force_tile<D, POT, UNIFORM, UW, KK, PR>;                                                       \
        if (!(attr_dev_mask & (1 << (c->device & 31)))) {                                                           \
            HIPCHK(hipFuncSetAttribute((const void *)kfn, hipFuncAttributeMaxDynamicSharedMemorySize,               \
                                       (int)(160 * 1024 - 2048)));                                                  \
            attr_dev_mask |= 1 << (c->device & 31);                                                                 \
        }                                                                                                           \
        kfn<<<nb, MD_TILE, lds_bytes, c->stream>>>(n, s, c->pp, rows16, c->maxn, rowmax, halo_p, halo_cap,          \
                                                   halo_cnt, dt, c->partials.p, nb, c->scal.p, step,                \
                                                   c->nlist16_in.p, c->nmax_tile_in.p, rin * rin,                   \
                                                   c->dbg_stamps.p, hin_p, c->hcap_in, c->halo_in_count.p);         \
    } while (0)
    prof_begin(c, prune_step ? 3 : 0);
    if (c->use_tiles) {
        if (prune_step) {
            if (want_uw)
                LT(true, true, true);
            else
                LT(false, true, true);
        } else if (want_uw) {
            if (kick)
                LT(true, true, false);
            else
                LT(true, false, false);
        } else {
            if (kick)
                LT(false, true, false);
            else
                LT(false, false, false);
        }
    } else if (want_uw) {
        if (kick)
            LF(true, true);
        else
            LF(true, false);
    } else {
        if (kick)
            LF(false, true);
        else
            LF(false, false);
    }
    prof_end(c);
#undef LF
#undef LT
    if (prune_step) {
        c->inner_valid = true;
        c->steps_since_prune = 0;
        c->st_prunes++;
    }
}

void launch_force_custom(md_ctx *c, int dim, bool want_uw, bool kick, double dt, int step)
{
    if (!c->rtc) throw HipError("custom potential selected but no compiled module (md_set_potential_source)");
    int n = (int)c->n;
    DevState s = c->dev(c->cur);
    int nb = c->nblk;
    prof_begin(c);
    if (c->use_tiles && c->tile_lds <= 64 * 1024) {
        const uint16_t *l16 = c->nlist16.p;
        int maxn = c->maxn;
        const int32_t *nmt = c->nmax_tile.p;
        const uint32_t *halo = c->halo.p;
        int hcap = c->hcap;
        const int32_t *hc = c->halo_count.p;
        double *part = c->partials.p;
        Scalars *sc = c->scal.p;
        uint16_t *rin = nullptr;
        int32_t *nin = nullptr;
        double rin2 = 0.0;
        long long *stamps = nullptr;
        uint32_t *hin = nullptr;
        int hcap_in = 0;
        int32_t *hinc = nullptr;
        void *args[] = {&n, &s, &c->pp, &l16, &maxn, &nmt, &halo, &hcap, &hc, &dt, &part, &nb, &sc, &step, &rin, &nin, &rin2, &stamps,
                        &hin, &hcap_in, &hinc};
        HIPCHK(hipModuleLaunchKernel(c->rtc->tile[dim - 2][want_uw][kick], nb, 1, 1, MD_TILE, 1, 1,
                                     (unsigned)c->tile_lds, c->stream, args, nullptr));
    } else {
        if (!c->have_nlist32) throw HipError("custom potential: halo too large for LDS and no 32-bit rows (set MDHIP_NO_FUSED_BUILD=1)");
        const uint32_t *l32 = c->nlist.p;
        int maxn = c->maxn;
        const int32_t *nmt = c->nmax_tile.p;
        double *part = c->partials.p;
        const Scalars *sc = c->scal.p;
        void *args[] = {&n, &s, &c->pp, &l32, &maxn, &nmt, &dt, &part, &nb, &sc, &step};
        HIPCHK(hipModuleLaunchKernel(c->rtc->global[dim - 2][want_uw][kick], nb, 1, 1, MD_BLOCK, 1, 1, 0, c->stream,
                                     args, nullptr));
    }
    prof_end(c);
}

template <int D>
void launch_force_d(md_ctx *c, bool want_uw, bool kick, double dt, int step, int rows)
{
    bool u = c->uniform_sigma;
    switch (c->pot_kind) {
    case POT_LJ:
        if (u)
            launch_force_tpu<D, POT_LJ, true>(c, want_uw, kick, dt, step, rows);
        else
            launch_force_tpu<D, POT_LJ, false>(c, want_uw, kick, dt, step, rows);
        break;
    case POT_PSEUDOHS:
        if (u)
            launch_force_tpu<D, POT_PSEUDOHS, true>(c, want_uw, kick, dt, step, rows);
        else
            launch_force_tpu<D, POT_PSEUDOHS, false>(c, want_uw, kick, dt, step, rows);
        break;
    case POT_POLYDISPERSE:
        launch_force_tpu<D, POT_POLYDISPERSE, false>(c, want_uw, kick, dt, step, rows);
        break;
    case POT_LJ_MOD:
        launch_force_tpu<D, POT_LJ_MOD, false>(c, want_uw, kick, dt, step, rows);
        break;
    case POT_CUSTOM:
        launch_force_custom(c, D, want_uw, kick, dt, step);
        break;
    default:
        throw HipError("potential kind not available (custom potentials need md_set_potential_source)");
    }
}

void launch_force(md_ctx *c, bool want_uw, bool kick, double dt, int step, int rows = 0)
{
    if (c->dim == 3)
        launch_force_d<3>(c, want_uw, kick, dt, step, rows);
    else
        launch_force_d<2>(c, want_uw, kick, dt, step, rows);
}

void launch_kickdrift(md_ctx *c, bool nvt, double dt, bool check, int step, BussiSrc bs = BussiSrc{})
{
    int n = (int)c->n;
    DevState s = c->dev(c->cur);
    int nb = c->nblk;
    double skin_half = check ? 0.5 * c->skin : INFINITY;
    double inner_half = check ? (c->inner_valid ? 0.5 * c->inner_skin : 0.5 * c->skin) : INFINITY;
    int use_d1 = c->inner_valid ? 1 : 0;
    prof_begin(c, 1);
    if (c->dim == 3) {
        if (nvt)
            k_kickdrift<3, true><<<nb, MD_BLOCK, 0, c->stream>>>(n, s, dt, skin_half, inner_half, use_d1, c->scal.p, step,
                                                                 bs);
        else
            k_kickdrift<3, false><<<nb, MD_BLOCK, 0, c->stream>>>(n, s, dt, skin_half, inner_half, use_d1, c->scal.p, step,
                                                                 bs);
    } else {
        if (nvt)
            k_kickdrift<2, true><<<nb, MD_BLOCK, 0, c->stream>>>(n, s, dt, skin_half, inner_half, use_d1, c->scal.p, step,
                                                                 bs);
        else
            k_kickdrift<2, false><<<nb, MD_BLOCK, 0, c->stream>>>(n, s, dt, skin_half, inner_half, use_d1, c->scal.p, step,
                                                                 bs);
    }
    prof_end(c);
}

void launch_ghost_update(md_ctx *c, int step)
{
    if (c->nghost == 0 || c->virtual_ghosts) return;
    DevState s = c->dev(c->cur);
    int nb = nblocks(c->nghost);
    if (c->dim == 3)
        k_ghost_update<3><<<nb, MD_BLOCK, 0, c->stream>>>((int)c->n, (int)c->nghost, s, c->grid, c->gowner.p,
                                                          c->gcode.p, c->scal.p, step);
    else
        k_ghost_update<2><<<nb, MD_BLOCK, 0, c->stream>>>((int)c->n, (int)c->nghost, s, c->grid, c->gowner.p,
                                                          c->gcode.p, c->scal.p, step);
}

void launch_finalize(md_ctx *c, bool want_uw, bool nvt, double nf, double term1, int step)
{
    k_finalize<<<1, 1024, 0, c->stream>>>(c->nblk, c->partials.p, want_uw ? 1 : 0, nvt ? 1 : 0, nf, term1, c->d_kt.p,
                                          c->d_r1.p, c->d_r2.p, c->scal.p, step);
}

bool fused_available(md_ctx *c)
{
    return c->allow_fused && c->use_tiles && c->virtual_ghosts && !c->dom.on && c->pot_kind != POT_CUSTOM && c->skin > 0.0;
}

bool fused_uniform(md_ctx *c)
{
    return c->uniform_sigma && c->pot_kind != POT_POLYDISPERSE && c->pot_kind != POT_LJ_MOD;
}

inline size_t rec_stride(md_ctx *c) { return c->dom.on ? (size_t)c->cap + 1 : (size_t)c->ncap; }

void fused_enter(md_ctx *c, double dt)
{
    int n = (int)c->n;
    const bool uni = fused_uniform(c);
    const size_t planes = uni ? 3 : 4;
    for (int w = 0; w < 2; ++w) c->rec[w].ensure(rec_stride(c) * planes);
    DevState s = c->dev(c->cur);
    double h2 = (dt * dt) / 2.0;
    c->fz_a = 0;
    if (c->nblk <= 0) return;
    if (c->dim == 3) {
        if (uni)
            k_fuse<3, true><<<c->nblk, MD_BLOCK, 0, c->stream>>>(n, s, c->rec[0].p, rec_stride(c), h2);
        else
            k_fuse<3, false><<<c->nblk, MD_BLOCK, 0, c->stream>>>(n, s, c->rec[0].p, rec_stride(c), h2);
    } else {
        if (uni)
            k_fuse<2, true><<<c->nblk, MD_BLOCK, 0, c->stream>>>(n, s, c->rec[0].p, rec_stride(c), h2);
        else
            k_fuse<2, false><<<c->nblk, MD_BLOCK, 0, c->stream>>>(n, s, c->rec[0].p, rec_stride(c), h2);
    }
    c->fz_a = 0;
}

void fused_leave(md_ctx *c, bool apply_scale)
{
    int n = (int)c->n;
    const bool uni = fused_uniform(c);
    if (c->fz_a) {
        StateBufs &a = c->sb[c->cur], &b = c->sb[c->cur ^ 1];
        std::swap(a.pos.p, b.pos.p);
        std::swap(a.pos.n, b.pos.n);
        for (int d = 0; d < c->dim; ++d) {
            std::swap(a.f[d].p, b.f[d].p);
            std::swap(a.f[d].n, b.f[d].n);
        }
    }
    DevState s = c->dev(c->cur);
    const double2 *rec = c->rec[c->fz_a].p;
    int ap = apply_scale ? 1 : 0;
    if (c->nblk <= 0) {
        c->fz_a = 0;
        return;
    }
    if (c->dim == 3) {
        if (uni)
            k_unfuse<3, true><<<c->nblk, MD_BLOCK, 0, c->stream>>>(n, s, rec, rec_stride(c), c->scal.p, ap);
        else
            k_unfuse<3, false><<<c->nblk, MD_BLOCK, 0, c->stream>>>(n, s, rec, rec_stride(c), c->scal.p, ap);
    } else {
        if (uni)
            k_unfuse<2, true><<<c->nblk, MD_BLOCK, 0, c->stream>>>(n, s, rec, rec_stride(c), c->scal.p, ap);
        else
            k_unfuse<2, false><<<c->nblk, MD_BLOCK, 0, c->stream>>>(n, s, rec, rec_stride(c), c->scal.p, ap);
    }
    c->fz_a = 0;
}

template <int D, int POT, bool UNIFORM>
void launch_step_tpu(md_ctx *c, bool want_uw, double dt, int step)
{
    int n = (int)c->n;
    int nb = c->nblk;
    bool prune_step = c->prune_on && !c->inner_valid;
    bool use_inner = c->inner_valid;
    const uint16_t *rows16 = use_inner ? c->nlist16_in.p : c->nlist16.p;
    const int32_t *rowmax = use_inner ? c->nmax_tile_in.p : c->nmax_tile.p;
    double skin_half = 0.5 * c->skin;
    double inner_half = use_inner ? 0.5 * c->inner_skin : 0.5 * c->skin;
    int use_d1 = use_inner ? 1 : 0;
    DevState s = c->dev(c->cur);
    double rin = c->rc + c->inner_skin;
    const bool whole = c->part.list == nullptr;
    hipStream_t lst = whole ? c->stream : c->part.stream;
    const int grid = whole ? nb : c->part.count;
    if (prune_step) {
        for (int d = 0; d < 3; ++d) s.x1[d] = c->x1[d].p;
        if (whole) k_reset_d1<<<1, 1, 0, c->stream>>>(c->scal.p, step - 1);
    }
    const uint32_t *halo_p = c->halo.p;
    int halo_cap = c->hcap;
    const int32_t *halo_cnt = c->halo_count.p;
    size_t lds_bytes = c->tile_lds;
    uint32_t *hin_p = nullptr;
    if (prune_step) {
        c->inner_halo_live = false;
    } else if (use_inner && c->inner_halo_live) {
        halo_p = c->halo_in.p;
        halo_cap = c->hcap_in;
        halo_cnt = c->halo_in_count.p;
        lds_bytes = c->tile_lds_in;
    }
    const int a = c->fz_a;
    StateBufs &A = c->sb[c->cur ^ a], &B = c->sb[c->cur ^ a ^ 1];
    StepBufs sbufs{};
    sbufs.recA = c->rec[a].p;
    sbufs.recB = c->rec[a ^ 1].p;
    sbufs.rstride = rec_stride(c);
    for (int d = 0; d < 3; ++d) {
        sbufs.fA[d] = A.f[d].p;
        sbufs.fB[d] = B.f[d].p;
    }
    sbufs.posB = B.pos.p;
#define LS(UW, PR)                                                                                                  \
    do {                                                                                                            \
        auto kfn = k_step_tile<D, POT, UNIFORM, UW, PR>;                                                            \
        static int attr_dev_mask = 0;                                                                               \
        if (!(attr_dev_mask & (1 << (c->device & 31)))) {                                                           \
            HIPCHK(hipFuncSetAttribute((const void *)kfn, hipFuncAttributeMaxDynamicSharedMemorySize,               \
                                       (int)(160 * 1024 - 2048)));                                                  \
            attr_dev_mask |= 1 << (c->device & 31);                                                                 \
        }                                                                                                           \
        if (grid > 0)                                                                                               \
            kfn<<<grid, MD_TILE, lds_bytes, lst>>>(n, s, sbufs, c->pp, rows16, c->maxn, rowmax, halo_p, halo_cap,   \
                                                   halo_cnt, dt, skin_half, inner_half, use_d1,                     \
                                                   c->partials.p, nb, c->scal.p, step, c->nlist16_in.p,             \
                                                   c->nmax_tile_in.p, rin * rin, c->dbg_stamps.p, hin_p,            \
                                                   c->hcap_in, c->halo_in_count.p, c->part.list);                   \
    } while (0)
    if (whole) prof_begin(c, prune_step ? 3 : 0);
    if (prune_step) {
        if (want_uw)
            LS(true, true);
        else
            LS(false, true);
    } else {
        if (want_uw)
            LS(true, false);
        else
            LS(false, false);
    }
    if (whole) prof_end(c);
#undef LS
    if (!whole && !c->part.last) return;
    c->fz_a ^= 1;
    if (prune_step) {
        c->inner_valid = true;
        c->steps_since_prune = 0;
        c->st_prunes++;
    }
}

template <int D>
void launch_step_d(md_ctx *c, bool want_uw, double dt, int step)
{
    bool u = c->uniform_sigma;
    switch (c->pot_kind) {
    case POT_LJ:
        if (u)
            launch_step_tpu<D, POT_LJ, true>(c, want_uw, dt, step);
        else
            launch_step_tpu<D, POT_LJ, false>(c, want_uw, dt, step);
        break;
    case POT_PSEUDOHS:
        if (u)
            launch_step_tpu<D, POT_PSEUDOHS, true>(c, want_uw, dt, step);
        else
            launch_step_tpu<D, POT_PSEUDOHS, false>(c, want_uw, dt, step);
        break;
    case POT_POLYDISPERSE:
        launch_step_tpu<D, POT_POLYDISPERSE, false>(c, want_uw, dt, step);
        break;
    case POT_LJ_MOD:
        launch_step_tpu<D, POT_LJ_MOD, false>(c, want_uw, dt, step);
        break;
    default:
        throw HipError("fused step loop: potential kind not available");
    }
}

void launch_step(md_ctx *c, bool want_uw, double dt, int step)
{
    if (c->dim == 3)
        launch_step_d<3>(c, want_uw, dt, step);
    else
        launch_step_d<2>(c, want_uw, dt, step);
}

Scalars read_scalars(md_ctx *c)
{
    Scalars h;
    HIPCHK(hipMemcpyAsync(&h, c->scal.p, sizeof(Scalars), hipMemcpyDeviceToHost, c->stream));
    HIPCHK(hipStreamSynchronize(c->stream));
    return h;
}

int fail(md_ctx *c, const char *what)
{
    if (c)
        c->err = what;
    else
        g_create_error = what;
    return 1;
}

}

struct FusedScope {
    md_ctx *c;
    bool done = false;
    ~FusedScope()
    {
        if (!done) c->state_invalid = true;
    }
};

inline void require_state(md_ctx *c, const char *who)
{
    if (c->state_invalid)
        throw HipError(std::string(who) + ": an earlier call failed inside the fused step loop and left the particle state "
                                          "incomplete; upload x, v and f again (md_upload) before going on");
}

#define API_BEGIN                                                                                                   \
    if (!ctx) return fail(nullptr, "null handle");                                                                  \
    try {                                                                                                           \
        HIPCHK(hipSetDevice(ctx->device));
#define API_END                                                                                                     \
    }                                                                                                               \
    catch (const std::exception &e) { return fail(ctx, e.what()); }                                                 \
    catch (...) { return fail(ctx, "unknown C++ exception"); }                                                      \
    return 0;

extern "C" {

const char *md_version(void) { return "mdhip 0.1 gfx950"; }

const char *md_last_error(md_ctx *ctx) { return ctx ? ctx->err.c_str() : g_create_error.c_str(); }

static int create_common(int dim, int64_t n_global, int64_t n_cap, bool domain, int rank, int nranks,
                         const double *box, double list_cutoff, int device_id, md_ctx **out)
{
    if (!out) return fail(nullptr, "md_create: out is null");
    *out = nullptr;
    if (dim != 2 && dim != 3) return fail(nullptr, "md_create: dim must be 2 or 3");
    if (n_global < 2) return fail(nullptr, "md_create: need at least 2 particles");
    if (n_cap < 2) return fail(nullptr, "md_create: capacity must be at least 2");
    if (n_cap >= (int64_t)MD_VAL_SRC_MASK / 2)
        return fail(nullptr, "md_create: too many particles for one handle (limit 2^25)");
    if (n_global >= (1ll << 31)) return fail(nullptr, "md_create: particle ids must fit 31 bits");
    if (!box) return fail(nullptr, "md_create: box is null");
    if (!(list_cutoff > 0.0)) return fail(nullptr, "md_create: list_cutoff must be positive");
    if (domain && (nranks < 1 || rank < 0 || rank >= nranks))
        return fail(nullptr, "md_create_domain: need nranks >= 1 and 0 <= rank < nranks");
    CellGeom cg;
    if (const char *why = cell_geometry(dim, box, cg)) return fail(nullptr, why);
    if (cg.tric && domain)
        return fail(nullptr, "md_create_domain: only orthorhombic (diagonal) unit cells are supported by the slab decomposition");
    md_ctx *ctx = nullptr;
    try {
        int ndev = 0;
        hipError_t e = hipGetDeviceCount(&ndev);
        if (e != hipSuccess || ndev == 0) return fail(nullptr, "md_create: no HIP device available (libmdhip has no CPU fallback)");
        ctx = new md_ctx();
        if (device_id < 0) HIPCHK(hipGetDevice(&device_id));
        if (device_id >= ndev) throw HipError("md_create: device_id out of range");
        ctx->device = device_id;
        HIPCHK(hipSetDevice(device_id));
        if (domain) {
            int plo = 0, phi = 0;
            HIPCHK(hipDeviceGetStreamPriorityRange(&plo, &phi));
            HIPCHK(hipStreamCreateWithPriority(&ctx->stream, hipStreamNonBlocking, phi));
        } else {
            HIPCHK(hipStreamCreateWithFlags(&ctx->stream, hipStreamNonBlocking));
        }
        ctx->own_stream = ctx->stream;
        ctx->dim = dim;
        ctx->n_global = n_global;
        ctx->ncap = n_cap;
        ctx->n = domain ? 0 : n_cap;
        for (int c = 0; c < dim; ++c) ctx->L[c] = box[c * dim + c];
        ctx->tric = cg.tric;
        for (int c = 0; c < 9; ++c) {
            ctx->A[c] = cg.A[c];
            ctx->Ainv[c] = cg.Ainv[c];
        }
        for (int c = 0; c < 3; ++c) ctx->perp[c] = cg.perp[c];
        ctx->volume = cg.volume;
        ctx->rc = list_cutoff;
        if (domain) {
            ctx->dom.on = true;
            ctx->skin_req = 0.4;
            ctx->dom.rank = rank;
            ctx->dom.nranks = nranks;
            ctx->dom.xlo = ctx->L[0] * rank / nranks;
            ctx->dom.xhi = (rank == nranks - 1) ? ctx->L[0] : ctx->L[0] * (rank + 1) / nranks;
        }
        if (const char *e = getenv("MDHIP_NO_TILES")) ctx->allow_tiles = !(e[0] == '1');
        if (const char *e = getenv("MDHIP_NO_FUSED_BUILD")) ctx->allow_fused_build = !(e[0] == '1');
        if (const char *e = getenv("MDHIP_INNER_SKIN")) ctx->inner_skin_req = atof(e);
        if (const char *e = getenv("MDHIP_NO_FUSED_STEP")) ctx->allow_fused = !(e[0] == '1');
        ctx->allow_inner_halo = false;
        if (const char *e = getenv("MDHIP_INNER_HALO")) ctx->allow_inner_halo = (e[0] == '1');
        ctx->pot_kind = POT_LJ;
        ctx->pp.p[0] = 1.0;
        ctx->pp.p[1] = 1.0;
        ctx->pp.p[2] = 2.5;
        configure_grid(ctx);
        configure_potential(ctx);
        double frac = 1.0;
        for (int c = 0; c < dim; ++c) frac *= (double)ctx->grid.ncx[c] / ctx->grid.nc[c];
        int64_t gcap = (int64_t)((frac - 1.0) * 1.3 * n_cap) + 4096;
        ctx->cap = n_cap + gcap;
        alloc_state(ctx, 0, ctx->cap);
        alloc_state(ctx, 1, ctx->cap);
        int64_t n = n_cap;
        ctx->nimg.alloc(ctx->cap + 2);
        ctx->img_off.alloc(ctx->cap + 2);
        HIPCHK(hipMemsetAsync(ctx->nimg.p, 0, sizeof(int32_t) * (ctx->cap + 2), ctx->stream));
        ctx->newslot.alloc(ctx->cap + 1);
        ctx->keys_in.alloc(ctx->cap);
        ctx->keys_out.alloc(ctx->cap);
        ctx->vals_in.alloc(ctx->cap);
        ctx->vals_out.alloc(ctx->cap);
        ctx->gsrc.alloc(ctx->cap + 1);
        ctx->gcode.alloc(ctx->cap + 1);
        ctx->gowner.alloc(ctx->cap + 1);
        ctx->nblk = nblocks(ctx->n);
        int nblk_cap = nblocks(n);
        ctx->ntiles = (int64_t)nblk_cap * (MD_BLOCK / 64);
        ctx->nneigh.alloc(n);
        ctx->nmax_tile.alloc(ctx->ntiles);
        double dens = (double)n_global;
        dens /= ctx->volume;
        double vol = (dim == 3) ? 4.18879020478639 * ctx->rl * ctx->rl * ctx->rl : 3.14159265358979 * ctx->rl * ctx->rl;
        int maxn = (int)(dens * vol * 1.35) + 24;
        ctx->maxn = (maxn + 3) & ~3;
        ctx->nlist.alloc((size_t)ctx->ntiles * ctx->maxn * 64);
        ctx->nlist16.alloc((size_t)ctx->ntiles * ctx->maxn * 64);
        ctx->halo.alloc((size_t)nblk_cap * ctx->hcap);
        ctx->halo_count.alloc(nblk_cap);
        if (getenv("MDHIP_STAMPS")) ctx->dbg_stamps.alloc((size_t)nblk_cap * 32);
        ctx->partials.alloc((size_t)3 * nblk_cap);
        HIPCHK(hipMemsetAsync(ctx->partials.p, 0, sizeof(double) * 3 * nblk_cap, ctx->stream));
        ctx->scal.alloc(1);
        Scalars h{};
        h.scale = 1.0;
        h.first_viol = MD_NO_VIOLATION;
        HIPCHK(hipMemcpyAsync(ctx->scal.p, &h, sizeof h, hipMemcpyHostToDevice, ctx->stream));
        ctx->d_kt.alloc(1);
        ctx->d_r1.alloc(1);
        ctx->d_r2.alloc(1);
        if (domain) {
            int64_t rec_cap = n_cap / 2 + 8192;
            ctx->dom.alive.alloc(2 * ctx->cap + 2);
            ctx->dom.counters.alloc(8);
            for (int sd = 0; sd < 2; ++sd) {
                ctx->dom.sbuf[sd].alloc((size_t)rec_cap * MD_MIG_REC);
                ctx->dom.rbuf[sd].alloc((size_t)rec_cap * MD_MIG_REC);
                ctx->dom.hs_src[sd].alloc(rec_cap);
                ctx->dom.send_slot[sd].alloc(rec_cap);
            }
            ctx->dom.xh_slot.alloc(2 * rec_cap);
        }
        for (int w = 0; w < 2; ++w)
            k_init_state<<<nblocks(ctx->cap + 1), MD_BLOCK, 0, ctx->stream>>>((int)n, ctx->cap, ctx->dev(w), dim);
        HIPCHK(hipGetLastError());
        HIPCHK(hipStreamSynchronize(ctx->stream));
    } catch (const std::exception &e) {
        g_create_error = e.what();
        delete ctx;
        return 1;
    }
    *out = ctx;
    return 0;
}

int md_create(int dim, int64_t n_particles, const double *box, double list_cutoff, int device_id, md_ctx **out)
{
    return create_common(dim, n_particles, n_particles, false, 0, 1, box, list_cutoff, device_id, out);
}

int md_create_domain(int dim, int64_t n_global, int64_t n_cap, const double *box, double list_cutoff,
                     int device_id, int rank, int nranks, md_ctx **out)
{
    return create_common(dim, n_global, n_cap, true, rank, nranks, box, list_cutoff, device_id, out);
}

static void dom_p2p_teardown(md_ctx *c);

int md_destroy(md_ctx *ctx)
{
    if (!ctx) return 0;
    (void)hipSetDevice(ctx->device);
    if (ctx->stream) {
        (void)hipStreamSynchronize(ctx->stream);
        (void)hipStreamDestroy(ctx->own_stream);
        if (ctx->copy_stream) (void)hipStreamDestroy(ctx->copy_stream);
        if (ctx->ev_snap_ready) (void)hipEventDestroy(ctx->ev_snap_ready);
        if (ctx->ev_snap_copied) (void)hipEventDestroy(ctx->ev_snap_copied);
        if (ctx->pin_x) (void)hipHostFree(ctx->pin_x);
        if (ctx->pin_i) (void)hipHostFree(ctx->pin_i);
    }
    delete ctx->rtc;
    ctx->rtc = nullptr;
    if (ctx->dom.stream_i) {
        (void)hipStreamSynchronize(ctx->dom.stream_i);
        (void)hipStreamDestroy(ctx->dom.stream_i);
        (void)hipEventDestroy(ctx->dom.ev_go);
        (void)hipEventDestroy(ctx->dom.ev_int);
    }
    dom_p2p_teardown(ctx);
    if (ctx->dom.comm && g_rccl.CommDestroy) (void)g_rccl.CommDestroy(ctx->dom.comm);
    ctx->dom.comm = nullptr;
    for (auto &p : ctx->prof_ev) {
        (void)hipEventDestroy(p.first);
        (void)hipEventDestroy(p.second);
    }
    delete ctx;
    return 0;
}

int md_set_potential(md_ctx *ctx, int kind, const double *params, int nparams)
{
    API_BEGIN
    if (kind != MD_POT_LJ && kind != MD_POT_PSEUDOHS && kind != MD_POT_POLYDISPERSE && kind != MD_POT_LJ_MODIFIED)
        throw HipError("md_set_potential: unknown potential kind");
    if (nparams < 0 || nparams > 8 || (nparams > 0 && !params)) throw HipError("md_set_potential: bad params");
    int need = (kind == MD_POT_LJ) ? 3 : (kind == MD_POT_PSEUDOHS ? 1 : (kind == MD_POT_LJ_MODIFIED ? 5 : 2));
    if (nparams < need) throw HipError("md_set_potential: too few parameters for this kind");
    if ((kind == MD_POT_LJ || kind == MD_POT_LJ_MODIFIED) && !(std::isfinite(params[2]) && params[2] > 0.0))
        throw HipError("md_set_potential: r_cut must be finite and > 0");
    for (int i = 0; i < 8; ++i) ctx->pp.p[i] = (i < nparams) ? params[i] : 0.0;
    if (kind == MD_POT_LJ_MODIFIED) {
        double eps = params[0], sg = params[1], rc = params[2];
        int mode = (int)params[3];
        if (mode < 0 || mode > 2) throw HipError("md_set_potential: MD_POT_LJ_MODIFIED mode must be 0, 1 or 2");
        if (mode == 2 && !(params[4] < rc)) throw HipError("md_set_potential: XPLOR needs r_on < r_cut");
        double s = sg / rc, s2 = s * s, s6 = s2 * s2 * s2, s12 = s6 * s6;
        ctx->pp.p[5] = 4.0 * eps * (s12 - s6);
        ctx->pp.p[6] = 24.0 * eps * (2.0 * s12 - s6) / rc;
    }
    ctx->pot_kind = kind;
    ctx->list_valid = false;
    configure_potential(ctx);
    API_END
}

int md_set_potential_source(md_ctx *ctx, const char *hip_src, const char *entry_name, const double *params,
                            int nparams)
{
    API_BEGIN
    if (!hip_src || !entry_name || !entry_name[0]) throw HipError("md_set_potential_source: source and entry name are required");
    if (nparams < 0 || nparams > 8 || (nparams > 0 && !params)) throw HipError("md_set_potential_source: at most 8 parameters");
    for (const char *q = entry_name; *q; ++q)
        if (!((*q >= 'a' && *q <= 'z') || (*q >= 'A' && *q <= 'Z') || (*q >= '0' && *q <= '9') || *q == '_'))
// ... 1137 lines not shown
    API_END
}

int md_run_brownian(md_ctx *ctx, int64_t nsteps, double dt, double ktemp, uint64_t seed, int64_t first_step,
                    int64_t virial_every, double *out)
{
    API_BEGIN
    require_state(ctx, "md_run_brownian");
    if (ctx->dom.on) throw HipError("md_run_brownian: not available on a slab-decomposition handle");
    if (nsteps < 0 || nsteps > 0x3ffffff0) throw HipError("md_run_brownian: bad nsteps");
    if (!(dt > 0.0) || !(ktemp > 0.0)) throw HipError("md_run_brownian: need dt > 0 and kT > 0");
    if (virial_every < 1) virial_every = 10;
    hipStream_t st = ctx->stream;
    ctx->brown_acc.ensure(2);
    HIPCHK(hipMemsetAsync(ctx->brown_acc.p, 0, 2 * sizeof(double), st));
    const double sigma = std::sqrt(2.0 * dt);
    ctx->list_valid = false;
    int64_t s = 0;
    while (s < nsteps) {
        if (!ctx->list_valid) rebuild(ctx);
        int64_t chunk_end = std::min<int64_t>(nsteps, s + 32);
        for (int64_t t = s; t < chunk_end; ++t) {
            int64_t g = first_step + t;
            bool sample = (g % virial_every) == 0;
            bool want = sample || t == nsteps - 1;
            launch_force(ctx, want, false, 0.0, (int)t);
            if (want)
                k_brownian_sums<<<1, 1024, 0, st>>>(ctx->nblk, ctx->partials.p, sample ? 1 : 0, ctx->brown_acc.p, ctx->scal.p,
                                                    (int)t);
            DevState sd = ctx->dev(ctx->cur);
            if (ctx->dim == 3)
                k_brownian_move<3><<<ctx->nblk, MD_BLOCK, 0, st>>>((int)ctx->n, sd, dt, ktemp, sigma, seed, g,
                                                                   0.5 * ctx->skin, ctx->scal.p, (int)t);
            else
                k_brownian_move<2><<<ctx->nblk, MD_BLOCK, 0, st>>>((int)ctx->n, sd, dt, ktemp, sigma, seed, g,
                                                                   0.5 * ctx->skin, ctx->scal.p, (int)t);
        }
        HIPCHK(hipGetLastError());
        Scalars h = read_scalars(ctx);
        if (h.first_viol <= chunk_end) {
            s = h.first_viol;
            ctx->list_valid = false;
            if (s < nsteps) ctx->st_viol++;
        } else {
            s = chunk_end;
        }
    }
    k_reset_viol<<<1, 1, 0, st>>>(ctx->scal.p);
    Scalars h = read_scalars(ctx);
    double acc[2];
    HIPCHK(hipMemcpyAsync(acc, ctx->brown_acc.p, sizeof acc, hipMemcpyDeviceToHost, st));
    HIPCHK(hipStreamSynchronize(st));
    if (out) {
        out[0] = h.U;
        out[1] = h.W;
        out[2] = acc[0];
        out[3] = acc[1];
    }
    ctx->list_valid = false;
    ctx->st_steps += nsteps;
    API_END
}

int md_kinetic(md_ctx *ctx, double *kinetic)
{
    API_BEGIN
    require_state(ctx, "md_kinetic");
    DevState s = ctx->dev(ctx->cur);
    if (ctx->dim == 3)
        k_ke_partials<3><<<ctx->nblk, MD_BLOCK, 0, ctx->stream>>>((int)ctx->n, s, ctx->partials.p);
    else
        k_ke_partials<2><<<ctx->nblk, MD_BLOCK, 0, ctx->stream>>>((int)ctx->n, s, ctx->partials.p);
    launch_finalize(ctx, false, false, 1.0, 0.0, -1);
    HIPCHK(hipGetLastError());
    Scalars h = read_scalars(ctx);
    if (kinetic) *kinetic = h.K;
    API_END
}

int md_scale_velocities(md_ctx *ctx, double sfac)
{
    API_BEGIN
    require_state(ctx, "md_scale_velocities");
    DevState s = ctx->dev(ctx->cur);
    if (ctx->dim == 3)
        k_scale_v<3><<<ctx->nblk, MD_BLOCK, 0, ctx->stream>>>((int)ctx->n, s, ctx->scal.p, sfac, 0);
    else
        k_scale_v<2><<<ctx->nblk, MD_BLOCK, 0, ctx->stream>>>((int)ctx->n, s, ctx->scal.p, sfac, 0);
    HIPCHK(hipGetLastError());
    HIPCHK(hipStreamSynchronize(ctx->stream));
    API_END
}

int md_profile(md_ctx *ctx, int enable)
{
    API_BEGIN
    prof_collect(ctx);
    ctx->prof = enable != 0;
    ctx->prof_stride = enable > 1 ? enable : 1;
    ctx->prof_seen[0] = ctx->prof_seen[1] = 0;
    if (enable) {
        ctx->prof_ms_acc = 0.0;
        ctx->prof_launch_acc = 0;
        ctx->prof_kd_ms_acc = 0.0;
        ctx->prof_kd_launch_acc = 0;
        ctx->prof_prune_acc = 0;
        ctx->prof_prune_ms_acc = 0.0;
        ctx->prof_rebuild_acc = 0;
        ctx->prof_rebuild_ms_acc = 0.0;
    }
    API_END
}

int md_get_stats(md_ctx *ctx, md_stats *out)
{
    API_BEGIN
    if (!out) throw HipError("md_get_stats: out is null");
    prof_collect(ctx);
    out->steps = ctx->st_steps;
    out->rebuilds = ctx->st_rebuilds;
    out->violations = ctx->st_viol;
    out->n_ghost = ctx->nghost;
    out->max_neighbors = ctx->maxn;
    out->avg_neighbors = 0.0;
    if (ctx->list_valid) {
        std::vector<int32_t> h((size_t)ctx->n);
        HIPCHK(hipMemcpyAsync(h.data(), ctx->nneigh.p, sizeof(int32_t) * ctx->n, hipMemcpyDeviceToHost, ctx->stream));
        HIPCHK(hipStreamSynchronize(ctx->stream));
        double sum = 0.0;
        for (int32_t v : h) sum += v;
        out->avg_neighbors = sum / (double)ctx->n;
    }
    out->prunes = ctx->st_prunes;
    out->max_halo = ctx->use_tiles ? ctx->hstride : 0;
    out->tiled = ctx->use_tiles ? 1 : 0;
    out->force_launches = ctx->prof_launch_acc;
    out->force_ms = ctx->prof_ms_acc;
    out->kickdrift_launches = ctx->prof_kd_launch_acc;
    out->kickdrift_ms = ctx->prof_kd_ms_acc;
    out->fused = ctx->last_run_fused ? 1 : 0;
    out->walked_outer = out->walked_inner = 0;
    if (ctx->list_valid) {
        const int64_t nw = (ctx->n + 63) / 64;
        std::vector<int32_t> h((size_t)nw);
        HIPCHK(hipMemcpyAsync(h.data(), ctx->nmax_tile.p, sizeof(int32_t) * nw, hipMemcpyDeviceToHost, ctx->stream));
        HIPCHK(hipStreamSynchronize(ctx->stream));
        for (int32_t v : h) out->walked_outer += 64 * (int64_t)v;
        if (ctx->inner_valid) {
            HIPCHK(hipMemcpyAsync(h.data(), ctx->nmax_tile_in.p, sizeof(int32_t) * nw, hipMemcpyDeviceToHost, ctx->stream));
            HIPCHK(hipStreamSynchronize(ctx->stream));
            for (int32_t v : h) out->walked_inner += 64 * (int64_t)v;
        }
    }
    out->prune_launches_timed = ctx->prof_prune_acc;
    out->prune_ms = ctx->prof_prune_ms_acc;
    out->rebuilds_timed = ctx->prof_rebuild_acc;
    out->rebuild_ms = ctx->prof_rebuild_ms_acc;
    out->fused_build = (ctx->list_valid && ctx->use_tiles && !ctx->have_nlist32) ? 1 : 0;
    API_END
}


namespace {
void dom_require(md_ctx *c)
{
    if (!c->dom.on) throw HipError("this handle was not created with md_create_domain");
}
DomCounters dom_read_counters(md_ctx *c)
{
    DomCounters h;
    HIPCHK(hipMemcpyAsync(&h, c->dom.counters.p, sizeof h, hipMemcpyDeviceToHost, c->stream));
    HIPCHK(hipStreamSynchronize(c->stream));
    if (h.error & 1) throw HipError("a particle moved by more than one slab between list builds");
    if (h.error & 2) throw HipError("slab exchange buffer overflow (raise n_cap)");
    return h;
}
}

int md_dom_set_uniform(md_ctx *ctx, int uniform, double sigma)
{
    API_BEGIN
    dom_require(ctx);
    ctx->uniform_sigma = uniform != 0;
    ctx->sigma_u = sigma;
    configure_potential(ctx);
    ctx->list_valid = false;
    API_END
}

int md_dom_upload(md_ctx *ctx, int64_t n_own, const int32_t *ids, const double *x, const double *v, const double *f,
                  const int32_t *images, const double *diameters)
{
    API_BEGIN
    if (x && v && f) ctx->state_invalid = false;
    dom_require(ctx);
    if (n_own < 0 || n_own > ctx->ncap) throw HipError("md_dom_upload: n_own exceeds the handle's capacity");
    if (n_own > 0 && (!ids || !x)) throw HipError("md_dom_upload: ids and x are required");
    size_t nd = (size_t)n_own * ctx->dim;
    hipStream_t st = ctx->stream;
    DBuf<int32_t> d_ids;
    d_ids.alloc(n_own + 1);
    ctx->io_x.ensure(nd + 1);
    ctx->io_v.ensure(nd + 1);
    ctx->io_f.ensure(nd + 1);
    ctx->io_i.ensure(nd + 1);
    ctx->io_d.ensure(n_own + 1);
    if (n_own > 0) {
        HIPCHK(hipMemcpyAsync(d_ids.p, ids, n_own * sizeof(int32_t), hipMemcpyHostToDevice, st));
        HIPCHK(hipMemcpyAsync(ctx->io_x.p, x, nd * sizeof(double), hipMemcpyHostToDevice, st));
        if (v) HIPCHK(hipMemcpyAsync(ctx->io_v.p, v, nd * sizeof(double), hipMemcpyHostToDevice, st));
        if (f) HIPCHK(hipMemcpyAsync(ctx->io_f.p, f, nd * sizeof(double), hipMemcpyHostToDevice, st));
        if (images) HIPCHK(hipMemcpyAsync(ctx->io_i.p, images, nd * sizeof(int32_t), hipMemcpyHostToDevice, st));
        if (diameters) HIPCHK(hipMemcpyAsync(ctx->io_d.p, diameters, n_own * sizeof(double), hipMemcpyHostToDevice, st));
        DevState s = ctx->dev(ctx->cur);
        int nb = nblocks(n_own);
        if (ctx->dim == 3)
            k_import_local<3><<<nb, MD_BLOCK, 0, st>>>((int)n_own, s, d_ids.p, ctx->io_x.p, v ? ctx->io_v.p : nullptr,
                                                       f ? ctx->io_f.p : nullptr, images ? ctx->io_i.p : nullptr,
                                                       diameters ? ctx->io_d.p : nullptr);
        else
            k_import_local<2><<<nb, MD_BLOCK, 0, st>>>((int)n_own, s, d_ids.p, ctx->io_x.p, v ? ctx->io_v.p : nullptr,
                                                       f ? ctx->io_f.p : nullptr, images ? ctx->io_i.p : nullptr,
                                                       diameters ? ctx->io_d.p : nullptr);
        HIPCHK(hipGetLastError());
    }
    HIPCHK(hipStreamSynchronize(st));
    ctx->n = n_own;
    ctx->nblk = nblocks(n_own);
    ctx->src_count = n_own;
    ctx->list_valid = false;
    API_END
}

int md_dom_download(md_ctx *ctx, int64_t cap, int64_t *n_own, int32_t *ids, double *x, double *v, double *f,
                    int32_t *images)
{
    API_BEGIN
    require_state(ctx, "md_dom_download");
    dom_require(ctx);
    if (n_own) *n_own = ctx->n;
    if (cap < ctx->n) throw HipError("md_dom_download: output capacity is smaller than the owned count");
    int64_t n = ctx->n;
    if (n == 0) return 0;
    size_t nd = (size_t)n * ctx->dim;
    hipStream_t st = ctx->stream;
    DBuf<int32_t> d_ids;
    d_ids.alloc(n);
    ctx->io_x.ensure(nd);
    ctx->io_v.ensure(nd);
    ctx->io_f.ensure(nd);
    ctx->io_i.ensure(nd);
    DevState s = ctx->dev(ctx->cur);
    if (ctx->dim == 3)
        k_export_local<3><<<nblocks(n), MD_BLOCK, 0, st>>>((int)n, s, ctx->grid, d_ids.p, ctx->io_x.p, ctx->io_v.p,
                                                           ctx->io_f.p, ctx->io_i.p);
    else
        k_export_local<2><<<nblocks(n), MD_BLOCK, 0, st>>>((int)n, s, ctx->grid, d_ids.p, ctx->io_x.p, ctx->io_v.p,
                                                           ctx->io_f.p, ctx->io_i.p);
    HIPCHK(hipGetLastError());
    if (ids) HIPCHK(hipMemcpyAsync(ids, d_ids.p, n * sizeof(int32_t), hipMemcpyDeviceToHost, st));
    if (x) HIPCHK(hipMemcpyAsync(x, ctx->io_x.p, nd * sizeof(double), hipMemcpyDeviceToHost, st));
    if (v) HIPCHK(hipMemcpyAsync(v, ctx->io_v.p, nd * sizeof(double), hipMemcpyDeviceToHost, st));
    if (f) HIPCHK(hipMemcpyAsync(f, ctx->io_f.p, nd * sizeof(double), hipMemcpyDeviceToHost, st));
    if (images) HIPCHK(hipMemcpyAsync(images, ctx->io_i.p, nd * sizeof(int32_t), hipMemcpyDeviceToHost, st));
    HIPCHK(hipStreamSynchronize(st));
    API_END
}

int md_dom_migrate_pack(md_ctx *ctx, int64_t *nsend)
{
    API_BEGIN
    dom_require(ctx);
    auto &d = ctx->dom;
    hipStream_t st = ctx->stream;
    d.n_old = ctx->n;
    d.n_arr = 0;
    d.n_xh = 0;
    HIPCHK(hipMemsetAsync(d.counters.p, 0, 8 * sizeof(int32_t), st));
    int cap_rec = (int)(d.sbuf[0].n / MD_MIG_REC);
    double inv_w = (double)d.nranks / ctx->L[0];
    DevState s = ctx->dev(ctx->cur);
    if (d.n_old > 0) {
        if (ctx->dim == 3)
            k_dom_classify<3><<<nblocks(d.n_old), MD_BLOCK, 0, st>>>((int)d.n_old, s, ctx->grid, d.xlo, d.xhi, inv_w,
                                                                     d.rank, d.nranks, d.alive.p, d.sbuf[0].p,
                                                                     d.sbuf[1].p, cap_rec, (DomCounters *)d.counters.p);
        else
            k_dom_classify<2><<<nblocks(d.n_old), MD_BLOCK, 0, st>>>((int)d.n_old, s, ctx->grid, d.xlo, d.xhi, inv_w,
                                                                     d.rank, d.nranks, d.alive.p, d.sbuf[0].p,
                                                                     d.sbuf[1].p, cap_rec, (DomCounters *)d.counters.p);
        HIPCHK(hipGetLastError());
    }
    DomCounters h = dom_read_counters(ctx);
    d.nsend_mig[0] = h.mig[0];
    d.nsend_mig[1] = h.mig[1];
    if (nsend) {
        nsend[0] = h.mig[0];
        nsend[1] = h.mig[1];
    }
    ctx->list_valid = false;
    API_END
}

int md_dom_set_step_buffers(md_ctx *ctx, void *send_left, void *send_right, void *recv_left, void *recv_right,
                            int64_t capacity_doubles)
{
    API_BEGIN
    dom_require(ctx);
    ctx->dom.ext_send[0] = (double *)send_left;
    ctx->dom.ext_send[1] = (double *)send_right;
    ctx->dom.ext_recv[0] = (double *)recv_left;
// ... 1192 lines not shown
```

### moleculardynamics/jl_amd/device.py

```python
import ctypes as C

import numpy as np

from . import _lib
from ._lib import MdhipError, MdStats


def _dp(a):
    return None if a is None else a.ctypes.data_as(C.POINTER(C.c_double))


def _ip(a):
    return None if a is None else a.ctypes.data_as(C.POINTER(C.c_int32))


def _f64(a, shape=None):
    if a is None:
        return None
    a = np.ascontiguousarray(a, dtype=np.float64)
    if shape is not None and a.shape != shape:
        raise ValueError(f"expected array of shape {shape}, got {a.shape}")
    return a


# ... 58 lines not shown
        if im is not None and im.shape != shp:
            raise ValueError("images must have shape (N, d)")
        d = _f64(diameters, (self.n,))
        self._chk(self._L.md_upload(self._h, _dp(x), _dp(v), _dp(f), _ip(im), _dp(d)))

    def download(self):
        shp = (self.n, self.dim)
        x, v, f = np.empty(shp), np.empty(shp), np.empty(shp)
        im = np.empty(shp, dtype=np.int32)
        self._chk(self._L.md_download(self._h, _dp(x), _dp(v), _dp(f), _ip(im)))
        return x, v, f, im

    def snapshot_begin(self):
        self._chk(self._L.md_snapshot_begin(self._h))

    def snapshot_end(self):
        shp = (self.n, self.dim)
        x = np.empty(shp)
        im = np.empty(shp, dtype=np.int32)
        self._chk(self._L.md_snapshot_end(self._h, _dp(x), _ip(im)))
        return x, im

    def compute_forces(self):
        u, w = C.c_double(), C.c_double()
        self._chk(self._L.md_compute_forces(self._h, C.byref(u), C.byref(w)))
        return u.value, w.value

    def neighbor_pairs(self):
        cnt = C.c_int64()
        self._chk(self._L.md_neighbor_pairs(self._h, None, 0, C.byref(cnt)))
        out = np.empty((max(cnt.value, 1), 2), dtype=np.int32)
        cnt2 = C.c_int64()
        self._chk(self._L.md_neighbor_pairs(self._h, _ip(out), cnt.value, C.byref(cnt2)))
        if cnt2.value != cnt.value:
            raise MdhipError("pair count changed between calls")
        out = out[: cnt.value]
        order = np.lexsort((out[:, 1], out[:, 0]))
        return out[order]

    def run(self, nsteps, dt, ensemble=_lib.MD_NVE, tau=0.0, nf=None, ktemp=None, r1=None, r2=None, thermo=True):
        nf = float(self.dim * (self.n - 1.0)) if nf is None else float(nf)
        kt, a1, a2 = _f64(ktemp), _f64(r1), _f64(r2)
        for a in (kt, a1, a2):
            if a is not None and a.size < nsteps:
                raise ValueError("per-step thermostat arrays are shorter than nsteps")
        uwk = np.zeros(3)
        self._chk(self._L.md_run(self._h, int(nsteps), float(dt), int(ensemble), float(tau), nf, _dp(kt), _dp(a1),
                                 _dp(a2), _dp(uwk) if thermo else None))
        return (uwk[0], uwk[1], uwk[2]) if thermo else None

    def fire_minimize(self, max_steps=10000, tol=1e-6, dt_initial=0.01, dt_max=0.1, alpha0=0.1, f_inc=1.2, f_dec=0.2,
                      nmin=5):
        st, cv = C.c_int64(), C.c_int()
        en, fr = C.c_double(), C.c_double()
        self._chk(self._L.md_fire_minimize(self._h, int(max_steps), float(tol), float(dt_initial), float(dt_max),
                                           float(alpha0), float(f_inc), float(f_dec), int(nmin), C.byref(st), C.byref(cv),
                                           C.byref(en), C.byref(fr)))
        return dict(steps=st.value, converged=bool(cv.value), energy=en.value, f_rms=fr.value)

    def run_brownian(self, nsteps, dt, ktemp, seed, first_step=0, virial_every=10):
        out = np.zeros(4)
        self._chk(self._L.md_run_brownian(self._h, int(nsteps), float(dt), float(ktemp), int(seed), int(first_step),
                                          int(virial_every), _dp(out)))
        return dict(U=out[0], W=out[1], virial_sum=out[2], virial_count=out[3])

    def kinetic(self):
        k = C.c_double()
        self._chk(self._L.md_kinetic(self._h, C.byref(k)))
        return k.value

    def scale_velocities(self, s):
        self._chk(self._L.md_scale_velocities(self._h, float(s)))

    def rdf_setup(self, r_max, nbins):
        self._chk(self._L.md_rdf_setup(self._h, float(r_max), int(nbins)))
        self._rdf_nbins = int(nbins)

    def rdf_sample(self):
        self._chk(self._L.md_rdf_sample(self._h))

    def rdf_read(self):
        counts = np.zeros(max(getattr(self, "_rdf_nbins", 0), 1), dtype=np.int64)
        ns = C.c_int64()
        self._chk(self._L.md_rdf_read(self._h, counts.ctypes.data_as(C.POINTER(C.c_int64)), C.byref(ns)))
        return counts[: getattr(self, "_rdf_nbins", 0)], ns.value

    def rdf_reset(self):
        self._chk(self._L.md_rdf_reset(self._h))

    def dyn_setup(self, nslots, nrows, q=(), r_max=0.0, nbins=0):
        qa = np.ascontiguousarray(q, dtype=np.float64).reshape(-1)
        self._chk(self._L.md_dyn_setup(self._h, int(nslots), int(nrows), _dp(qa) if qa.size else None, int(qa.size),
                                       float(r_max), int(nbins)))
        self._dyn_shape = (int(nrows), int(qa.size), int(nbins))

    def dyn_origin(self, slot):
        self._chk(self._L.md_dyn_origin(self._h, int(slot)))

    def dyn_sample(self, slots, rows):
        s = np.ascontiguousarray(slots, dtype=np.int32).reshape(-1)
        r = np.ascontiguousarray(rows, dtype=np.int32).reshape(-1)
        if s.shape != r.shape:
            raise ValueError("slots and rows must have the same length")
        self._chk(self._L.md_dyn_sample(self._h, _ip(s), _ip(r), int(s.size)))

    def dyn_read(self):
        nrows, nq, nbins = getattr(self, "_dyn_shape", (0, 0, 0))
        ns = np.zeros(max(nrows, 1), dtype=np.int64)
        sums = np.zeros((max(nrows, 1), 2 + nq))
        hist = np.zeros((max(nrows, 1), max(nbins, 1)), dtype=np.int64)
        i64 = C.POINTER(C.c_int64)
        self._chk(self._L.md_dyn_read(self._h, ns.ctypes.data_as(i64), _dp(sums), hist.ctypes.data_as(i64)))
        return ns[:nrows], sums[:nrows], hist[:nrows, :nbins]

    def dyn_reset(self):
        self._chk(self._L.md_dyn_reset(self._h))

    def sq_setup(self, n, nslots=0, nrows=0):
        na = np.ascontiguousarray(n, dtype=np.int32)
        if na.ndim != 2 or na.shape[1] != self.dim:
            raise ValueError(f"n must have shape (nvec, {self.dim})")
        self._chk(self._L.md_sq_setup(self._h, _ip(na) if na.size else None, int(na.shape[0]), int(nslots), int(nrows)))
        self._sq_shape = (int(na.shape[0]), int(nrows))

    def sq_sample(self, static=True, slots=(), rows=(), origin=None):
        s = np.ascontiguousarray(slots, dtype=np.int32).reshape(-1)
        r = np.ascontiguousarray(rows, dtype=np.int32).reshape(-1)
        if s.shape != r.shape:
            raise ValueError("slots and rows must have the same length")
        self._chk(self._L.md_sq_sample(self._h, 1 if static else 0, _ip(s) if s.size else None, _ip(r) if r.size else None,
                                       int(s.size), -1 if origin is None else int(origin)))

    def sq_rho(self):
        nvec, _ = getattr(self, "_sq_shape", (0, 0))
        out = np.zeros((max(nvec, 1), 2))
        self._chk(self._L.md_sq_rho(self._h, _dp(out)))
        return out[:nvec].copy().view(np.complex128).reshape(nvec)

    def sq_read(self):
        nvec, nrows = getattr(self, "_sq_shape", (0, 0))
        nst = C.c_int64()
        s2 = np.zeros(max(nvec, 1))
        ns = np.zeros(max(nrows, 1), dtype=np.int64)
        corr = np.zeros((max(nrows, 1), max(nvec, 1)))
        self._chk(self._L.md_sq_read(self._h, C.byref(nst), _dp(s2), ns.ctypes.data_as(C.POINTER(C.c_int64)), _dp(corr)))
        return nst.value, s2[:nvec], ns[:nrows], corr[:nrows, :nvec]

    def sq_reset(self):
        self._chk(self._L.md_sq_reset(self._h))

    def profile(self, enable=True):
        self._chk(self._L.md_profile(self._h, int(enable)))

    def stats(self):
        s = MdStats()
        self._chk(self._L.md_get_stats(self._h, C.byref(s)))
        return {k: getattr(s, k) for k, _ in MdStats._fields_}
```

Before: 6.631 billion particle-steps/s.

## Sort lanes by inner-row length within tiles and round rows to two

During prune steps each tile ranks its particles by their previous inner-list length using an LDS counting sort. It then assigns them to wave slots so that particles with similar row lengths share a wave, and stores the lane permutation. Non-prune steps read this permutation, load particle state through it, walk a per-wave padded row length that is now rounded to 2 instead of 4 (with a new 2-wide tail block), and unpermute the reductions. The aim is less wasted padded pair work from wave-level max row length, at the cost of extra LDS, syncs, a permutation gather and scattered own-particle loads.

```diff
diff --git a/include/mdhip.h b/include/mdhip.h
--- a/include/mdhip.h
+++ b/include/mdhip.h
@@ -91,9 +91,11 @@
     int64_t rebuilds_timed;
     double rebuild_ms;
     int64_t fused_build;
+    int64_t lane_sort;
 } md_stats;
 int md_profile(md_ctx *ctx, int enable);
 int md_get_stats(md_ctx *ctx, md_stats *out);
+int md_debug_lane_map(md_ctx *ctx, void *lane_part , int32_t *nmax_in, int32_t *row_len, int64_t *ntiles);
 
 int md_create_domain(int dim, int64_t n_global, int64_t n_cap, const double *box, double list_cutoff,
                      int device_id, int rank, int nranks, md_ctx **out);
diff --git a/moleculardynamics/jl_amd/_lib.py b/moleculardynamics/jl_amd/_lib.py
--- a/moleculardynamics/jl_amd/_lib.py
+++ b/moleculardynamics/jl_amd/_lib.py
@@ -11,7 +11,7 @@
     "md_create", "md_destroy", "md_last_error", "md_set_potential", "md_set_potential_source", "md_set_skin",
     "md_set_inner_skin",
     "md_upload", "md_download", "md_snapshot_begin", "md_snapshot_end", "md_compute_forces", "md_neighbor_pairs", "md_run", "md_kinetic",
-    "md_scale_velocities", "md_profile", "md_get_stats", "md_version", "md_fire_minimize", "md_run_brownian",
+    "md_scale_velocities", "md_profile", "md_get_stats", "md_debug_lane_map", "md_version", "md_fire_minimize", "md_run_brownian",
     "md_create_domain", "md_dom_set_uniform", "md_dom_upload", "md_dom_download", "md_dom_migrate_pack",
     "md_dom_migrate_unpack", "md_dom_halo_pack", "md_dom_halo_unpack", "md_dom_build", "md_dom_get_sendbuf",
     "md_dom_put_recvbuf", "md_dom_set_step_buffers", "md_dom_step_begin", "md_dom_step_end", "md_dom_forces", "md_dom_set_scale",
@@ -31,7 +31,7 @@
                 ("kickdrift_launches", C.c_int64), ("kickdrift_ms", C.c_double), ("fused", C.c_int64),
                 ("walked_outer", C.c_int64), ("walked_inner", C.c_int64), ("prune_launches_timed", C.c_int64),
                 ("prune_ms", C.c_double), ("rebuilds_timed", C.c_int64), ("rebuild_ms", C.c_double),
-                ("fused_build", C.c_int64)]
+                ("fused_build", C.c_int64), ("lane_sort", C.c_int64)]
 
 
 class MdhipError(RuntimeError):
@@ -87,6 +87,8 @@
     L.md_profile.restype = C.c_int
     L.md_get_stats.argtypes = [vp, C.POINTER(MdStats)]
     L.md_get_stats.restype = C.c_int
+    L.md_debug_lane_map.argtypes = [vp, C.c_void_p, ip, ip, C.POINTER(C.c_int64)]
+    L.md_debug_lane_map.restype = C.c_int
     L.md_version.argtypes = []
     L.md_version.restype = C.c_char_p
     i64p = C.POINTER(C.c_int64)
diff --git a/moleculardynamics/jl_amd/csrc/md_kernels.hpp b/moleculardynamics/jl_amd/csrc/md_kernels.hpp
--- a/moleculardynamics/jl_amd/csrc/md_kernels.hpp
+++ b/moleculardynamics/jl_amd/csrc/md_kernels.hpp
@@ -26,6 +26,7 @@
     int32_t *id;
     double *x0[3];
     double *x1[3];
+    int32_t *cinp;
     double boxL[3];
     int tric;
     double cellA[9];
@@ -596,6 +597,7 @@
             sn.img[c][k] = so.img[c][src];
             sn.x0[c][k] = pos_get(p, c);
         }
+        sn.cinp[k] = so.cinp[src];
     } else {
         gsrc[k - n] = src;
         gcode[k - n] = code;
@@ -987,7 +989,7 @@
     }
 }
 
-template <int D, int POT, bool UNIFORM, bool WANT_UW, bool PRUNE>
+template <int D, int POT, bool UNIFORM, bool WANT_UW, bool PRUNE, bool TAIL2 = false>
 __device__ __forceinline__ void tile_pair_loop(const unsigned char *smem, const ushort4 *row4,
                                                ushort4 (&jn)[MD_UNROLL / 4], int m_lane, int H,
                                                const double4 &pi, const PotParams &pp, PruneRow &rin64,
@@ -1016,23 +1018,74 @@
         tile_pair_block<D, POT, UNIFORM, WANT_UW, PRUNE, MD_UNROLL>(smem, o, pi, pp, rin64, rin2, acc, cin, fx, fy, fz, us,
                                                                      ws, remap8);
     }
-    if (r < m) {
+    if (r < m && (!TAIL2 || r + 4 <= m)) {
         unsigned o[4] = {jn[0].x, jn[0].y, jn[0].z, jn[0].w};
         tile_pair_block<D, POT, UNIFORM, WANT_UW, PRUNE, 4>(smem, o, pi, pp, rin64, rin2, acc, cin, fx, fy, fz, us, ws,
                                                             remap8);
-    }
+        r += 4;
+        jn[0] = jn[1];
+    }
+    if constexpr (TAIL2) {
+        if (r < m) {
+            unsigned o[2] = {jn[0].x, jn[0].y};
+            tile_pair_block<D, POT, UNIFORM, WANT_UW, PRUNE, 2>(smem, o, pi, pp, rin64, rin2, acc, cin, fx, fy, fz, us, ws,
+                                                                remap8);
+        }
+    }
+}
+
+struct LaneSortLds {
+    unsigned char cnt[(MD_TILE / 64) * 256];
+    int scan[16];
+    int mw[MD_TILE / 64];
+};
+__device__ __forceinline__ int tile_lane_rank(int key, bool active, LaneSortLds &l)
+{
+    const int tid = threadIdx.x, lane = tid & 63, w = tid >> 6;
+    ((unsigned *)l.cnt)[tid] = 0u;
+    __syncthreads();
+    const int b = 255 - min(max(key, 0), 255);
+    int prefix = 0;
+    unsigned long long todo = __ballot(active);
+    while (todo) {
+        const int leader = __ffsll((long long)todo) - 1;
+        const int bv = __shfl(b, leader);
+        const bool mine = active && b == bv;
+        const unsigned long long msk = __ballot(mine);
+        if (mine) prefix = __popcll(msk & ((1ull << lane) - 1ull));
+        if (lane == leader) l.cnt[w * 256 + bv] = (unsigned char)__popcll(msk);
+        todo &= ~msk;
+    }
+    __syncthreads();
+    int c[MD_TILE / 64], tot = 0;
+#pragma unroll
+    for (int i = 0; i < MD_TILE / 64; ++i) {
+        c[i] = l.cnt[i * 256 + tid];
+        tot += c[i];
+    }
+    int all;
+    int base = block_excl_scan(tot, l.scan, &all);
+#pragma unroll
+    for (int i = 0; i < MD_TILE / 64; ++i) {
+        l.cnt[i * 256 + tid] = (unsigned char)base;
+        base += c[i];
+    }
+    __syncthreads();
+    return active ? (int)l.cnt[w * 256 + b] + prefix : tid;
 }
 
 template <int D, bool UNIFORM>
 __device__ __forceinline__ void tile_prune_tail(DevState &s, Scalars *sc, int H , int k, bool active, int lane, int wt,
                                                 const double4 &pi, PruneRow rin64, int32_t *nmax_in,
-                                                unsigned long long acc, int cin)
+                                                unsigned long long acc, int cin, int slot, int round, LaneSortLds &l)
 {
     constexpr int RS = UNIFORM ? 24 : 32;
     {
         const unsigned long long sent = (unsigned long long)(H * RS);
         const unsigned long long sent4 = sent | (sent << 16) | (sent << 32) | (sent << 48);
-        int mw = wave_max_i((cin + 3) & ~3);
+        atomicMax(&l.mw[slot >> 6], cin);
+        __syncthreads();
+        const int mw = (l.mw[slot >> 6] + round - 1) & ~(round - 1);
         int g = cin >> 2;
         if (cin & 3) {
             int p = cin & 3;
@@ -1040,8 +1093,9 @@
             rin64.off += 512u;
             ++g;
         }
-        for (; g < (mw >> 2); ++g, rin64.off += 512u) *(unsigned long long *)(rin64.base + rin64.off) = sent4;
-        if (lane == 0) nmax_in[wt] = mw;
+        for (; g < ((mw + 3) >> 2); ++g, rin64.off += 512u) *(unsigned long long *)(rin64.base + rin64.off) = sent4;
+        if (lane == 0) nmax_in[wt] = (l.mw[threadIdx.x >> 6] + round - 1) & ~(round - 1);
+        if (active) s.cinp[k] = cin;
         double dd = 0.0;
         if (active) {
 #pragma unroll
@@ -1144,6 +1198,24 @@
     return sh_hin;
 }
 
+template <bool WANT_K, bool WANT_UW>
+__device__ __forceinline__ void tile_unpermute(unsigned char *smem, int lp, double &ke, double &us, double &ws)
+{
+    double *pl = (double *)smem;
+    __syncthreads();
+    if constexpr (WANT_K) pl[lp] = ke;
+    if constexpr (WANT_UW) {
+        pl[MD_TILE + lp] = us;
+        pl[2 * MD_TILE + lp] = ws;
+    }
+    __syncthreads();
+    if constexpr (WANT_K) ke = pl[threadIdx.x];
+    if constexpr (WANT_UW) {
+        us = pl[MD_TILE + threadIdx.x];
+        ws = pl[2 * MD_TILE + threadIdx.x];
+    }
+}
+
 template <int D, int POT, bool UNIFORM, bool WANT_UW, bool KICK, bool PRUNE>
 __global__ void __launch_bounds__(MD_TILE)
     k_force_tile(int n, DevState s, PotParams pp, const uint16_t *__restrict__ nlist16, int maxn,
@@ -1151,7 +1223,8 @@
                  const int32_t *__restrict__ halo_count, double dt, double *__restrict__ partials, int nblk_total,
                  Scalars *__restrict__ sc, int step, uint16_t *__restrict__ rows_in, int32_t *__restrict__ nmax_in,
                  double rin2, long long *__restrict__ stamps = nullptr, uint32_t *__restrict__ halo_in = nullptr,
-                 int hcap_in = 0, int32_t *__restrict__ halo_in_count = nullptr)
+                 int hcap_in = 0, int32_t *__restrict__ halo_in_count = nullptr, unsigned char *__restrict__ lane_part = nullptr,
+                 int row_round = 4)
 {
 #define MD_SSTAMP(i)                                                                                   \
     do {                                                                                               \
@@ -1161,35 +1234,52 @@
     constexpr int RS = UNIFORM ? 24 : 32;
     extern __shared__ __attribute__((aligned(16))) unsigned char smem[];
     __shared__ double red[16];
+    __shared__ LaneSortLds lsl;
     if (sc->first_viol <= step) return;
     MD_SSTAMP(0);
     int bid = xcd_remap(blockIdx.x, gridDim.x);
     const double4 *__restrict__ P = s.pos;
     int H = halo_count[bid];
     const uint32_t *hl = halo + (size_t)bid * hcap;
-    int k = bid * MD_TILE + threadIdx.x;
+    const bool mapped = !PRUNE && lane_part != nullptr;
+    int lp = threadIdx.x;
+    if (mapped) lp = lane_part[(size_t)bid * MD_TILE + threadIdx.x];
+    int k = bid * MD_TILE + lp;
     bool active = k < n;
     int kk = active ? k : n - 1;
     int lane = threadIdx.x & 63;
     int wt = bid * (MD_TILE / 64) + (threadIdx.x >> 6);
     const ushort4 *row4 = (const ushort4 *)(nlist16 + ((size_t)wt * maxn) * 64) + lane;
-    PruneRow rin64;
-    rin64.base = PRUNE ? (unsigned char *)(rows_in + ((size_t)__builtin_amdgcn_readfirstlane(wt) * maxn) * 64) : nullptr;
-    rin64.off = (unsigned)lane * 8u;
     unsigned long long acc = 0ull;
     int cin = 0;
     int m = nmax_tile[wt];
-    double4 pi = P[kk];
+    double4 pi;
+    double v0[3] = {0.0, 0.0, 0.0};
+    auto load_own = [&]() {
+        pi = P[kk];
+        if constexpr (KICK) {
+#pragma unroll
+            for (int c = 0; c < D; ++c) v0[c] = s.v[c][kk];
+        }
+    };
+    if (!mapped) load_own();
     constexpr int G = MD_UNROLL / 4;
     ushort4 jn[G];
 #pragma unroll
     for (int g = 0; g < G; ++g) jn[g] = row4[(size_t)((4 * g < m) ? g : 0) * 64];
-    double v0[3] = {0.0, 0.0, 0.0};
-    if constexpr (KICK) {
-#pragma unroll
-        for (int c = 0; c < D; ++c) v0[c] = s.v[c][kk];
-    }
     MD_SSTAMP(1);
+    int slot = threadIdx.x;
+    PruneRow rin64;
+    rin64.base = nullptr;
+    if constexpr (PRUNE) {
+        if (threadIdx.x < MD_TILE / 64) lsl.mw[threadIdx.x] = 0;
+        if (lane_part) {
+            slot = tile_lane_rank(active ? s.cinp[kk] : 0, active, lsl);
+            lane_part[(size_t)bid * MD_TILE + slot] = (unsigned char)threadIdx.x;
+        }
+        rin64.base = (unsigned char *)(rows_in + ((size_t)(bid * (MD_TILE / 64) + (slot >> 6)) * maxn) * 64);
+    }
+    rin64.off = (unsigned)(slot & 63) * 8u;
     for (int h0 = 0; h0 <= H; h0 += 8 * MD_TILE) {
         uint32_t idx[8];
 #pragma unroll
@@ -1197,6 +1287,7 @@
             int h = h0 + i * MD_TILE + threadIdx.x;
             idx[i] = (h < H) ? hl[h] : 0xffffffffu;
         }
+        if (mapped && h0 == 0) load_own();
         double4 pr[8];
 #pragma unroll
         for (int i = 0; i < 8; ++i)
@@ -1230,9 +1321,9 @@
                                                 &remap8);
     }
     double fx = 0.0, fy = 0.0, fz = 0.0, us = 0.0, ws = 0.0;
-    tile_pair_loop<D, POT, UNIFORM, WANT_UW, PRUNE>(smem, row4, jn, m, H, pi, pp, rin64, rin2, acc, cin, fx, fy, fz, us, ws, remap8);
+    tile_pair_loop<D, POT, UNIFORM, WANT_UW, PRUNE, !PRUNE>(smem, row4, jn, m, H, pi, pp, rin64, rin2, acc, cin, fx, fy, fz, us, ws, remap8);
     MD_SSTAMP(4);
-    if constexpr (PRUNE) tile_prune_tail<D, UNIFORM>(s, sc, Hsent, k, active, lane, wt, pi, rin64, nmax_in, acc, cin);
+    if constexpr (PRUNE) tile_prune_tail<D, UNIFORM>(s, sc, Hsent, k, active, lane, wt, pi, rin64, nmax_in, acc, cin, slot, row_round, lsl);
     double ke = 0.0;
     if (active) {
         s.f[0][k] = fx;
@@ -1254,6 +1345,7 @@
         us = 0.0;
         ws = 0.0;
     }
+    if (mapped) tile_unpermute<KICK, WANT_UW>(smem, lp, ke, us, ws);
     if constexpr (KICK) {
         double t = block_sum(ke, red);
         if (threadIdx.x == 0) partials[bid] = t;
@@ -1287,7 +1379,8 @@
                 double *__restrict__ partials, int nblk_total, Scalars *__restrict__ sc, int step,
                 uint16_t *__restrict__ rows_in, int32_t *__restrict__ nmax_in, double rin2,
                 long long *__restrict__ stamps, uint32_t *__restrict__ halo_in, int hcap_in,
-                int32_t *__restrict__ halo_in_count, const int32_t *__restrict__ tile_list = nullptr)
+                int32_t *__restrict__ halo_in_count, const int32_t *__restrict__ tile_list = nullptr,
+                unsigned char *__restrict__ lane_part = nullptr, int row_round = 4)
 {
 #define MD_SSTAMP(i)                                                                                   \
     do {                                                                                               \
@@ -1297,41 +1390,60 @@
     constexpr int RS = UNIFORM ? 24 : 32;
     extern __shared__ __attribute__((aligned(16))) unsigned char smem[];
     __shared__ double red[16];
+    __shared__ LaneSortLds lsl;
     if (sc->first_viol < step) return;
     MD_SSTAMP(0);
     int bid = xcd_remap(blockIdx.x, gridDim.x);
     if (tile_list) bid = tile_list[bid];
     int H = halo_count[bid];
     const uint32_t *hl = halo + (size_t)bid * hcap;
-    int k = bid * MD_TILE + threadIdx.x;
+    const bool mapped = !PRUNE && lane_part != nullptr;
+    int lp = threadIdx.x;
+    if (mapped) lp = lane_part[(size_t)bid * MD_TILE + threadIdx.x];
+    int k = bid * MD_TILE + lp;
     bool active = k < n;
     int kk = active ? k : n - 1;
     int lane = threadIdx.x & 63;
     int wt = bid * (MD_TILE / 64) + (threadIdx.x >> 6);
     const ushort4 *row4 = (const ushort4 *)(nlist16 + ((size_t)wt * maxn) * 64) + lane;
-    PruneRow rin64;
-    rin64.base = PRUNE ? (unsigned char *)(rows_in + ((size_t)__builtin_amdgcn_readfirstlane(wt) * maxn) * 64) : nullptr;
-    rin64.off = (unsigned)lane * 8u;
     unsigned long long acc = 0ull;
     int cin = 0;
     int m = nmax_tile[wt];
     const double alpha = sc->scale;
     const double adt = alpha * dt;
     const double2 *RA0 = sb.recA, *RA1 = RA0 + sb.rstride, *RA2 = RA1 + sb.rstride, *RA3 = RA2 + sb.rstride;
-    double2 a0 = RA0[kk], a1 = RA1[kk], a2 = RA2[kk];
+    double2 a0, a1, a2;
     double sig_own = pp.sig_u;
-    if constexpr (!UNIFORM) sig_own = RA3[kk].x;
     double fprev[3] = {0.0, 0.0, 0.0}, xr[3] = {0.0, 0.0, 0.0};
-#pragma unroll
-    for (int c = 0; c < D; ++c) {
-        fprev[c] = sb.fA[c][kk];
-        xr[c] = PRUNE ? s.x0[c][kk] : s.x1[c][kk];
-    }
+    auto load_own = [&]() {
+        a0 = RA0[kk];
+        a1 = RA1[kk];
+        a2 = RA2[kk];
+        if constexpr (!UNIFORM) sig_own = RA3[kk].x;
+#pragma unroll
+        for (int c = 0; c < D; ++c) {
+            fprev[c] = sb.fA[c][kk];
+            xr[c] = PRUNE ? s.x0[c][kk] : s.x1[c][kk];
+        }
+    };
+    if (!mapped) load_own();
     constexpr int G = MD_UNROLL / 4;
     ushort4 jn[G];
 #pragma unroll
     for (int g = 0; g < G; ++g) jn[g] = row4[(size_t)((4 * g < m) ? g : 0) * 64];
     MD_SSTAMP(1);
+    int slot = threadIdx.x;
+    PruneRow rin64;
+    rin64.base = nullptr;
+    if constexpr (PRUNE) {
+        if (threadIdx.x < MD_TILE / 64) lsl.mw[threadIdx.x] = 0;
+        if (lane_part) {
+            slot = tile_lane_rank(active ? s.cinp[kk] : 0, active, lsl);
+            lane_part[(size_t)bid * MD_TILE + slot] = (unsigned char)threadIdx.x;
+        }
+        rin64.base = (unsigned char *)(rows_in + ((size_t)(bid * (MD_TILE / 64) + (slot >> 6)) * maxn) * 64);
+    }
+    rin64.off = (unsigned)(slot & 63) * 8u;
 #ifndef MD_STAGE_NB
 #define MD_STAGE_NB ((!PRUNE && UNIFORM && !WANT_UW) ? 6 : 8)
 #endif
@@ -1343,6 +1455,7 @@
             int h = h0 + i * MD_TILE + threadIdx.x;
             idx[i] = (h < H) ? hl[h] : 0xffffffffu;
         }
+        if (mapped && h0 == 0) load_own();
         double2 r0[NB], r1[NB], r2[NB], r3[NB];
 #pragma unroll
         for (int i = 0; i < NB; ++i) {
@@ -1400,9 +1513,9 @@
     __syncthreads();
     MD_SSTAMP(3);
     double fx = 0.0, fy = 0.0, fz = 0.0, us = 0.0, ws = 0.0;
-    tile_pair_loop<D, POT, UNIFORM, WANT_UW, PRUNE>(smem, row4, jn, m, H, pi, pp, rin64, rin2, acc, cin, fx, fy, fz, us, ws, nullptr);
+    tile_pair_loop<D, POT, UNIFORM, WANT_UW, PRUNE, !PRUNE>(smem, row4, jn, m, H, pi, pp, rin64, rin2, acc, cin, fx, fy, fz, us, ws, nullptr);
     MD_SSTAMP(4);
-    if constexpr (PRUNE) tile_prune_tail<D, UNIFORM>(s, sc, H, k, active, lane, wt, pi, rin64, nmax_in, acc, cin);
+    if constexpr (PRUNE) tile_prune_tail<D, UNIFORM>(s, sc, H, k, active, lane, wt, pi, rin64, nmax_in, acc, cin, slot, row_round, lsl);
     double ke = 0.0;
     if (active) {
         const double fn[3] = {fx, fy, fz};
@@ -1424,6 +1537,7 @@
         us = 0.0;
         ws = 0.0;
     }
+    if (mapped) tile_unpermute<true, WANT_UW>(smem, lp, ke, us, ws);
     {
         double t = block_sum(ke, red);
         if (threadIdx.x == 0) partials[bid] = t;
diff --git a/moleculardynamics/jl_amd/csrc/mdhip.hip b/moleculardynamics/jl_amd/csrc/mdhip.hip
--- a/moleculardynamics/jl_amd/csrc/mdhip.hip
+++ b/moleculardynamics/jl_amd/csrc/mdhip.hip
@@ -71,6 +71,7 @@
     DBuf<double4> pos;
     DBuf<double> v[3], f[3], x0[3];
     DBuf<int32_t> img[3], id;
+    DBuf<int32_t> cinp;
 };
 
 inline int ceil_log2(uint64_t v)
@@ -204,6 +205,9 @@
     DBuf<double> x1[3];
     DBuf<uint16_t> nlist16_in;
     DBuf<int32_t> nmax_tile_in;
+    DBuf<uint8_t> lane_part;
+    bool lane_sort = true;
+    int row_round = 2;
     int64_t steps_since_prune = 0;
     DBuf<double2> rec[2];
     DBuf<uint32_t> halo_in;
@@ -308,6 +312,7 @@
             s.x1[c] = (inner_valid && x1[c].p) ? x1[c].p : b.x0[c].p;
         }
         s.id = b.id.p;
+        s.cinp = b.cinp.p;
         for (int c = 0; c < 3; ++c) s.boxL[c] = c < dim ? L[c] : 0.0;
         s.tric = tric;
         for (int c = 0; c < 9; ++c) s.cellA[c] = A[c];
@@ -358,6 +363,8 @@
         b.x0[d].alloc(c->ncap);
     }
     b.id.alloc(cap + 1);
+    b.cinp.alloc(c->ncap);
+    HIPCHK(hipMemsetAsync(b.cinp.p, 0, sizeof(int32_t) * b.cinp.n, c->stream));
 }
 
 struct CellGeom {
@@ -743,6 +750,7 @@
         for (int d = 0; d < c->dim; ++d) c->x1[d].ensure(c->ncap);
         c->nlist16_in.ensure((size_t)c->ntiles * c->maxn * 64);
         c->nmax_tile_in.ensure(c->ntiles);
+        if (c->lane_sort) c->lane_part.ensure((size_t)c->nblk * MD_TILE);
         const size_t target = (c->tile_rs == 24) ? (40 * 1024 - 256) : (53 * 1024);
         int cap_in = (int)std::min<size_t>((size_t)c->hstride, target / c->tile_rs - 1);
         if (c->dom.on || getenv("MDHIP_INNER_CAP_OUTER")) cap_in = c->hstride;
@@ -839,6 +847,8 @@
     }
     DevState s = c->dev(c->cur);
     double rin = c->rc + c->inner_skin;
+    uint8_t *lane_p = ((prune_step || use_inner) && c->lane_sort && c->use_tiles) ? c->lane_part.p : nullptr;
+    if (lane_p && use_inner) lds_bytes = std::max<size_t>(lds_bytes, 3 * MD_TILE * sizeof(double));
     if (prune_step) {
         for (int d = 0; d < 3; ++d) s.x1[d] = c->x1[d].p;
         k_reset_d1<<<1, 1, 0, c->stream>>>(c->scal.p, step);
@@ -859,7 +869,8 @@
         kfn<<<nb, MD_TILE, lds_bytes, c->stream>>>(n, s, c->pp, rows16, c->maxn, rowmax, halo_p, halo_cap,          \
                                                    halo_cnt, dt, c->partials.p, nb, c->scal.p, step,                \
                                                    c->nlist16_in.p, c->nmax_tile_in.p, rin * rin,                   \
-                                                   c->dbg_stamps.p, hin_p, c->hcap_in, c->halo_in_count.p);         \
+                                                   c->dbg_stamps.p, hin_p, c->hcap_in, c->halo_in_count.p, lane_p,  \
+                                                   c->row_round);                                                   \
     } while (0)
     prof_begin(c, prune_step ? 3 : 0);
     if (c->use_tiles) {
@@ -923,8 +934,10 @@
         uint32_t *hin = nullptr;
         int hcap_in = 0;
         int32_t *hinc = nullptr;
+        uint8_t *lane_p = nullptr;
+        int row_round = 4;
         void *args[] = {&n, &s, &c->pp, &l16, &maxn, &nmt, &halo, &hcap, &hc, &dt, &part, &nb, &sc, &step, &rin, &nin, &rin2, &stamps,
-                        &hin, &hcap_in, &hinc};
+                        &hin, &hcap_in, &hinc, &lane_p, &row_round};
         HIPCHK(hipModuleLaunchKernel(c->rtc->tile[dim - 2][want_uw][kick], nb, 1, 1, MD_TILE, 1, 1,
                                      (unsigned)c->tile_lds, c->stream, args, nullptr));
     } else {
@@ -1130,6 +1143,8 @@
         halo_cnt = c->halo_in_count.p;
         lds_bytes = c->tile_lds_in;
     }
+    uint8_t *lane_p = ((prune_step || use_inner) && c->lane_sort) ? c->lane_part.p : nullptr;
+    if (lane_p && use_inner) lds_bytes = std::max<size_t>(lds_bytes, 3 * MD_TILE * sizeof(double));
     const int a = c->fz_a;
     StateBufs &A = c->sb[c->cur ^ a], &B = c->sb[c->cur ^ a ^ 1];
     StepBufs sbufs{};
@@ -1155,7 +1170,8 @@
                                                    halo_cnt, dt, skin_half, inner_half, use_d1,                     \
                                                    c->partials.p, nb, c->scal.p, step, c->nlist16_in.p,             \
                                                    c->nmax_tile_in.p, rin * rin, c->dbg_stamps.p, hin_p,            \
-                                                   c->hcap_in, c->halo_in_count.p, c->part.list);                   \
+                                                   c->hcap_in, c->halo_in_count.p, c->part.list, lane_p,            \
+                                                   c->row_round);                                                   \
     } while (0)
     if (whole) prof_begin(c, prune_step ? 3 : 0);
     if (prune_step) {
@@ -1331,6 +1347,8 @@
         if (const char *e = getenv("MDHIP_NO_FUSED_STEP")) ctx->allow_fused = !(e[0] == '1');
         ctx->allow_inner_halo = false;
         if (const char *e = getenv("MDHIP_INNER_HALO")) ctx->allow_inner_halo = (e[0] == '1');
+        if (const char *e = getenv("MDHIP_LANE_SORT")) ctx->lane_sort = !(e[0] == '0');
+        if (const char *e = getenv("MDHIP_ROW_ROUND")) ctx->row_round = (e[0] == '4') ? 4 : 2;
         ctx->pot_kind = POT_LJ;
         ctx->pp.p[0] = 1.0;
         ctx->pp.p[1] = 1.0;
@@ -2774,11 +2792,52 @@
             for (int32_t v : h) out->walked_inner += 64 * (int64_t)v;
         }
     }
+    if (getenv("MDHIP_ROWSTATS") && ctx->list_valid && ctx->prune_on && ctx->inner_valid) {
+        const int n = (int)ctx->n, nw = (n + 63) / 64, rr = ctx->row_round;
+        std::vector<int32_t> len((size_t)n), nm((size_t)nw);
+        HIPCHK(hipMemcpyAsync(len.data(), ctx->sb[ctx->cur].cinp.p, sizeof(int32_t) * n, hipMemcpyDeviceToHost, ctx->stream));
+        HIPCHK(hipMemcpyAsync(nm.data(), ctx->nmax_tile_in.p, sizeof(int32_t) * nw, hipMemcpyDeviceToHost, ctx->stream));
+        HIPCHK(hipStreamSynchronize(ctx->stream));
+        double mean = 0, walked = 0, exact = 0;
+        for (int i = 0; i < n; ++i) mean += len[i];
+        for (int w = 0; w < nw; ++w) walked += 64.0 * nm[w];
+        for (int t0 = 0; t0 < n; t0 += MD_TILE) {
+            std::vector<int> v(len.begin() + t0, len.begin() + std::min(n, t0 + MD_TILE));
+            std::sort(v.begin(), v.end(), std::greater<int>());
+            for (size_t w = 0; w * 64 < v.size(); ++w) exact += 64.0 * ((v[w * 64] + rr - 1) & ~(rr - 1));
+        }
+        fprintf(stderr, "[mdhip] inner rows (lane sort %d, round %d): mean %.2f  walked %.2f  walked-if-exactly-sorted %.2f\n",
+                ctx->lane_sort ? 1 : 0, rr, mean / n, walked / n, exact / n);
+    }
     out->prune_launches_timed = ctx->prof_prune_acc;
     out->prune_ms = ctx->prof_prune_ms_acc;
     out->rebuilds_timed = ctx->prof_rebuild_acc;
     out->rebuild_ms = ctx->prof_rebuild_ms_acc;
     out->fused_build = (ctx->list_valid && ctx->use_tiles && !ctx->have_nlist32) ? 1 : 0;
+    out->lane_sort = (ctx->prune_on && ctx->lane_sort) ? 1 : 0;
+    API_END
+}
+
+int md_debug_lane_map(md_ctx *ctx, void *lane_part_out, int32_t *nmax_in, int32_t *row_len, int64_t *ntiles)
+{
+    API_BEGIN
+    if (!ntiles) throw HipError("md_debug_lane_map: ntiles is null");
+    *ntiles = 0;
+    if (!ctx->list_valid || !ctx->prune_on || !ctx->inner_valid) return 0;
+    const int64_t nt = ctx->nblk;
+    hipStream_t st = ctx->stream;
+    if (uint8_t *lane_part = (uint8_t *)lane_part_out) {
+        if (ctx->lane_sort)
+            HIPCHK(hipMemcpyAsync(lane_part, ctx->lane_part.p, (size_t)nt * MD_TILE, hipMemcpyDeviceToHost, st));
+        else
+            for (int64_t i = 0; i < nt * MD_TILE; ++i) lane_part[i] = (uint8_t)(i & (MD_TILE - 1));
+    }
+    if (nmax_in)
+        HIPCHK(hipMemcpyAsync(nmax_in, ctx->nmax_tile_in.p, sizeof(int32_t) * nt * (MD_TILE / 64), hipMemcpyDeviceToHost, st));
+    if (row_len)
+        HIPCHK(hipMemcpyAsync(row_len, ctx->sb[ctx->cur].cinp.p, sizeof(int32_t) * ctx->n, hipMemcpyDeviceToHost, st));
+    HIPCHK(hipStreamSynchronize(st));
+    *ntiles = nt;
     API_END
 }
 
diff --git a/moleculardynamics/jl_amd/device.py b/moleculardynamics/jl_amd/device.py
--- a/moleculardynamics/jl_amd/device.py
+++ b/moleculardynamics/jl_amd/device.py
@@ -234,6 +234,17 @@
     def profile(self, enable=True):
         self._chk(self._L.md_profile(self._h, int(enable)))
 
+    def lane_map(self):
+        nt = (self.n + 255) // 256
+        lp = np.zeros((nt, 256), dtype=np.uint8)
+        nm = np.zeros((nt, 4), dtype=np.int32)
+        rl = np.zeros(self.n, dtype=np.int32)
+        cnt = C.c_int64()
+        self._chk(self._L.md_debug_lane_map(self._h, lp.ctypes.data_as(C.c_void_p), _ip(nm), _ip(rl), C.byref(cnt)))
+        if cnt.value == 0:
+            return None
+        return lp[: cnt.value], nm[: cnt.value], rl
+
     def stats(self):
         s = MdStats()
         self._chk(self._L.md_get_stats(self._h, C.byref(s)))
```

Result: slower. 6.119 billion particle-steps/s (-7.7%).
